# shyam196/egc

Measured on AMD Instinct MI355X. Metric: EGC-M layer fwd edges/sec on ogbn-arxiv; achieved HBM GB/s vs roofline, higher is better.
Workload: dtype f32; 1 GPU; ogbn-arxiv-shaped full graph: N=169343, heavy-tailed symmetrised E_in=2329056 (+N self loops => E_eff=2498399), EGC-M d=128 H=8 B=4 aggrs=sum+mean+max+symnorm, CSR cached; n_nodes=169343, e_in=2329056, e_eff=2498399, layer=EGConv, parallelism=single GPU

## Files before the change

egc_amd/_C.py:

```python
from __future__ import annotations

import ctypes as C
import os

_LIB_PATH = os.environ.get("EGC_HIP_LIB") or os.path.join(os.path.dirname(os.path.abspath(__file__)), "lib",
                                                         "libegc_hip.so")
_lib = None

EGC_MAX_AGGRS = 8
LONG_ROW_THRESHOLD = 64
LONG_ROW_CHUNK = 256

AGGR_SUM, AGGR_MEAN, AGGR_MAX, AGGR_MIN, AGGR_VAR, AGGR_STD, AGGR_SYMNORM = range(7)
SET_RAW, SET_LOOPED = 0, 1
LAYOUT_HBA, LAYOUT_HAB = 0, 1
ACT_NONE, ACT_SOFTMAX, ACT_SIGMOID, ACT_HARDTANH = range(4)
READOUT_SUM, READOUT_MEAN, READOUT_MAX = range(3)
SOFTMAX_MAX_CLASSES = 1024
TYPED_MAX_RELATIONS = 8
TOKEN_HEAD_MAX_SEQ = 8
TOKEN_HEAD_SLAB = 64
TOKEN_HEAD_MAX_IN = 384
MPNN_ADD, MPNN_MEAN, MPNN_MAX = range(3)
PNA_SUM, PNA_MEAN, PNA_MIN, PNA_MAX, PNA_VAR, PNA_STD = range(6)
PNA_IDENTITY, PNA_AMPLIFICATION, PNA_ATTENUATION, PNA_LINEAR, PNA_INVERSE_LINEAR = range(5)
NBR_SUM, NBR_MEAN, NBR_MEAN_T, NBR_SYM = range(4)

_STATUS = {1: "EGC_ERR_INVALID", 2: "EGC_ERR_WORKSPACE", 3: "EGC_ERR_HIP", 4: "EGC_ERR_UNSUPPORTED"}


class EgcGraph(C.Structure):
    _fields_ = [
        ("n_nodes", C.c_int64), ("n_edges", C.c_int64),
        ("rowptr", C.c_void_p), ("col", C.c_void_p), ("edge_id", C.c_void_p),
        ("dis_raw", C.c_void_p), ("dis_looped", C.c_void_p),
        ("max_index", C.c_void_p), ("plan", C.c_void_p), ("n_chunks", C.c_int64),
        ("n_src_rows", C.c_int64), ("edge_dis_raw", C.c_void_p), ("edge_dis_looped", C.c_void_p),
    ]


class EgcLayer(C.Structure):
    _fields_ = [
        ("in_channels", C.c_int32), ("out_channels", C.c_int32), ("num_heads", C.c_int32),
        ("num_bases", C.c_int32), ("num_aggrs", C.c_int32), ("aggrs", C.c_int32 * EGC_MAX_AGGRS),
        ("agg_set", C.c_int32), ("sym_set", C.c_int32), ("loops_all_nodes", C.c_int32),
        ("weight_layout", C.c_int32), ("weight_act", C.c_int32), ("basis_stride", C.c_int32),
    ]


_ENV_DATA = getattr(os.environ, "_data", None)


def env_flag(name: str) -> bool:
    if _ENV_DATA is not None:
        v = _ENV_DATA.get(name.encode())
        return v is not None and v not in (b"", b"0")
    return os.environ.get(name, "0") not in ("", "0")


class EgcPost(C.Structure):
    _fields_ = [("scale", C.c_void_p), ("shift", C.c_void_p), ("residual", C.c_void_p), ("relu", C.c_int32)]


class EgcTypedRel(C.Structure):
    _fields_ = [("rowptr", C.c_void_p), ("col", C.c_void_p), ("pre_rowptr", C.c_void_p), ("in_", C.c_void_p),
                ("n_edges", C.c_int64), ("n_in_rows", C.c_int64), ("ld_in", C.c_int32), ("out_col", C.c_int32),
                ("post_mean", C.c_int32), ("reserved", C.c_int32)]


SYMBOLS = {
    "egc_plan_ints": (C.c_int64, [C.c_int64, C.c_int64]),
    "egc_coo_to_csr_workspace_bytes": (C.c_size_t, [C.c_int64, C.c_int64]),
    "egc_coo_to_csr": (C.c_int, [C.c_void_p, C.c_void_p, C.c_int64, C.c_int64, C.c_void_p, C.c_void_p,
                                 C.c_void_p, C.c_void_p, C.c_void_p, C.c_size_t, C.c_void_p]),
    "egc_coo_to_csr_checked": (C.c_int, [C.c_void_p, C.c_void_p, C.c_int64, C.c_int64, C.c_int64, C.c_void_p, C.c_void_p,
                                         C.c_void_p, C.c_void_p, C.c_void_p, C.c_void_p, C.c_void_p, C.c_size_t, C.c_void_p]),
    "egc_graph_build_workspace_bytes": (C.c_size_t, [C.c_int64, C.c_int64]),
    "egc_graph_build_scratch_bytes": (C.c_size_t, [C.c_int64]),
    "egc_graph_build": (C.c_int, [C.c_void_p, C.c_void_p, C.c_int64, C.c_int64, C.c_int64, C.c_void_p, C.c_void_p, C.c_void_p,
                                  C.c_void_p, C.c_void_p, C.c_void_p, C.c_void_p, C.c_void_p, C.c_void_p, C.c_void_p,
                                  C.c_void_p, C.c_void_p, C.c_size_t, C.c_void_p, C.c_size_t, C.c_void_p]),
    "egc_csr_edge_dis": (C.c_int, [C.c_int64, C.c_void_p, C.c_void_p, C.c_void_p, C.c_void_p, C.c_void_p, C.c_void_p]),
    "egc_csr_prepare": (C.c_int, [C.c_int64, C.c_int64, C.c_void_p, C.c_void_p, C.c_void_p, C.c_void_p,
                                  C.c_void_p, C.c_void_p]),
    "egc_bases_ld": (C.c_int32, [C.POINTER(EgcLayer)]),
    "egc_basis_transform_f32": (C.c_int, [C.c_void_p, C.c_void_p, C.c_void_p, C.c_int64, C.c_int32, C.c_int32,
                                          C.c_int32, C.c_void_p, C.c_int32, C.c_void_p, C.c_void_p]),
    "egc_basis_pack_bytes": (C.c_size_t, [C.c_int32, C.c_int32, C.c_int32]),
    "egc_basis_pack": (C.c_int, [C.c_void_p, C.c_int32, C.c_int32, C.c_int32, C.c_void_p, C.c_size_t, C.c_void_p]),
    "egc_layer_gemm_flags": (C.c_int32, [C.POINTER(EgcLayer)]),
    "egc_basis_pack_ex": (C.c_int, [C.c_void_p, C.c_int32, C.c_int32, C.c_int32, C.c_int32, C.c_void_p, C.c_size_t, C.c_void_p]),
    "egc_basis_transform_packed_ex": (C.c_int, [C.c_void_p, C.c_void_p, C.c_void_p, C.c_int64, C.c_int32, C.c_int32,
                                                C.c_int32, C.c_int32, C.c_void_p, C.c_int32, C.c_void_p, C.c_void_p]),
    "egc_basis_transform_packed_add": (C.c_int, [C.c_void_p, C.c_void_p, C.c_void_p, C.c_int64, C.c_int32, C.c_int32,
                                                 C.c_int32, C.c_int32, C.c_void_p, C.c_void_p, C.c_int32, C.c_void_p, C.c_void_p]),
    "egc_basis_pack_transposed": (C.c_int, [C.c_void_p, C.c_int64, C.c_int32, C.c_int32, C.c_int32, C.c_void_p, C.c_size_t,
                                            C.c_void_p]),
    "egc_basis_transform_packed": (C.c_int, [C.c_void_p, C.c_void_p, C.c_void_p, C.c_int64, C.c_int32, C.c_int32,
                                             C.c_int32, C.c_void_p, C.c_int32, C.c_void_p, C.c_void_p]),
    "egc_layer_forward_packed": (C.c_int, [C.POINTER(EgcGraph), C.POINTER(EgcLayer), C.c_void_p, C.c_void_p,
                                           C.c_void_p, C.c_void_p, C.c_void_p, C.c_int32, C.c_void_p, C.c_void_p,
                                           C.c_void_p, C.c_size_t, C.c_void_p]),
    "egc_aggregate_workspace_bytes": (C.c_size_t, [C.POINTER(EgcLayer), C.c_int64, C.c_int64]),
    "egc_aggregate_workspace_zero_bytes": (C.c_size_t, [C.POINTER(EgcLayer), C.c_int64, C.c_int64]),
    "egc_aggregate_workspace_bytes_for": (C.c_size_t, [C.POINTER(EgcLayer), C.POINTER(EgcGraph)]),
    "egc_aggregate_combine_f32": (C.c_int, [C.POINTER(EgcGraph), C.POINTER(EgcLayer), C.c_void_p, C.c_int32,
                                            C.c_void_p, C.c_void_p, C.c_void_p, C.c_void_p, C.c_void_p,
                                            C.c_void_p, C.c_size_t, C.c_void_p]),
    "egc_layer_forward_f32": (C.c_int, [C.POINTER(EgcGraph), C.POINTER(EgcLayer), C.c_void_p, C.c_void_p,
                                        C.c_void_p, C.c_void_p, C.c_void_p, C.c_int32, C.c_void_p, C.c_void_p,
                                        C.c_void_p, C.c_size_t, C.c_void_p]),
    "egc_backward_workspace_bytes": (C.c_size_t, [C.POINTER(EgcLayer), C.c_int64]),
    "egc_backward_workspace_bytes_for": (C.c_size_t, [C.POINTER(EgcLayer), C.POINTER(EgcGraph)]),
    "egc_aggregate_combine_rows_f32": (C.c_int, [C.POINTER(EgcGraph), C.POINTER(EgcLayer), C.c_void_p, C.c_int32,
                                                 C.c_void_p, C.c_void_p, C.c_void_p, C.c_int64, C.c_int64,
                                                 C.c_void_p, C.c_size_t, C.c_void_p]),
    "egc_aggregate_combine_post_f32": (C.c_int, [C.POINTER(EgcGraph), C.POINTER(EgcLayer), C.c_void_p, C.c_int32,
                                                 C.c_void_p, C.c_void_p, C.POINTER(EgcPost), C.c_void_p,
                                                 C.c_void_p, C.c_size_t, C.c_void_p]),
    "egc_aggregate_combine_strided_f32": (C.c_int, [C.POINTER(EgcGraph), C.POINTER(EgcLayer), C.c_void_p, C.c_int32,
                                                    C.c_void_p, C.c_int32, C.c_void_p, C.POINTER(EgcPost), C.c_void_p,
                                                    C.c_void_p, C.c_size_t, C.c_void_p]),
    "egc_weight_grad_workspace_bytes": (C.c_int64, [C.c_int64, C.c_int32, C.c_int32]),
    "egc_weight_grad_plan": (C.c_int, [C.c_int64, C.c_int32, C.c_int32, C.c_void_p]),
    "egc_weight_grad_ex_workspace_bytes": (C.c_int64, [C.c_int64, C.c_int32, C.c_int32, C.c_int32]),
    "egc_weight_grad_ex_f32": (C.c_int, [C.c_void_p, C.c_int64, C.c_void_p, C.c_int64, C.c_int64, C.c_int32, C.c_int32,
                                         C.c_void_p, C.c_void_p, C.c_void_p, C.c_int64, C.c_int32, C.c_void_p, C.c_void_p,
                                         C.c_int64, C.c_void_p]),
    "egc_weight_grad_params_f32": (C.c_int, [C.c_void_p, C.c_int64, C.c_void_p, C.c_int64, C.c_int64, C.c_int32, C.c_int32, C.c_int32,
                                             C.c_int32, C.c_int32, C.c_int32, C.c_int32, C.c_void_p, C.c_int32, C.c_void_p,
                                             C.c_void_p, C.c_void_p, C.c_void_p, C.c_int64, C.c_int32, C.c_void_p, C.c_void_p,
                                             C.c_int64, C.c_void_p]),
    "egc_weight_grad_f32": (C.c_int, [C.c_void_p, C.c_int64, C.c_void_p, C.c_int64, C.c_int64, C.c_int32, C.c_int32,
                                      C.c_void_p, C.c_void_p, C.c_void_p, C.c_int64, C.c_void_p]),
    "egc_csr_transposed_coo": (C.c_int, [C.c_int64, C.c_int64, C.c_void_p, C.c_void_p, C.c_void_p, C.c_void_p, C.c_void_p]),
    "egc_column_moments_f64": (C.c_int, [C.c_void_p, C.c_void_p, C.c_void_p, C.c_void_p, C.c_int32, C.c_void_p, C.c_float,
                                         C.c_int64, C.c_int32, C.c_void_p, C.c_int32, C.c_void_p, C.c_void_p, C.c_void_p]),
    "egc_bn_forward_stats_f32": (C.c_int, [C.c_void_p, C.c_int64, C.c_int32, C.c_void_p, C.c_int32, C.c_void_p, C.c_void_p, C.c_void_p,
                                           C.c_void_p, C.c_double, C.c_void_p, C.c_void_p, C.c_void_p, C.c_void_p, C.c_double,
                                           C.c_void_p, C.c_void_p, C.c_void_p]),
    "egc_bn_backward_stats_f32": (C.c_int, [C.c_void_p, C.c_void_p, C.c_void_p, C.c_void_p, C.c_int32, C.c_void_p, C.c_float, C.c_int64,
                                            C.c_int32, C.c_void_p, C.c_int32, C.c_void_p, C.c_void_p, C.c_void_p, C.c_void_p,
                                            C.c_void_p, C.c_void_p]),
    "egc_bn_backward_stats_sums_f32": (C.c_int, [C.c_void_p, C.c_void_p, C.c_void_p, C.c_void_p, C.c_int32, C.c_void_p, C.c_float, C.c_int64,
                                                 C.c_int32, C.c_void_p, C.c_int32, C.c_void_p, C.c_void_p, C.c_void_p, C.c_void_p,
                                                 C.c_void_p, C.c_void_p, C.c_void_p]),
    "egc_bn_forward_finalize": (C.c_int, [C.c_void_p, C.c_int32, C.c_int32, C.c_int64, C.c_void_p, C.c_void_p, C.c_double,
                                          C.c_void_p, C.c_void_p, C.c_void_p, C.c_void_p, C.c_double, C.c_void_p, C.c_void_p,
                                          C.c_void_p]),
    "egc_bn_backward_finalize": (C.c_int, [C.c_void_p, C.c_int32, C.c_int32, C.c_int64, C.c_void_p, C.c_void_p, C.c_void_p,
                                           C.c_void_p, C.c_void_p]),
    "egc_affine_act_residual_f32": (C.c_int, [C.c_void_p, C.c_void_p, C.c_void_p, C.c_void_p, C.c_int32, C.c_void_p, C.c_float,
                                              C.c_int64, C.c_int32, C.c_void_p, C.c_void_p, C.c_void_p]),
    "egc_affine_act_backward_f32": (C.c_int, [C.c_void_p, C.c_void_p, C.c_void_p, C.c_void_p, C.c_int32, C.c_void_p, C.c_float,
                                              C.c_void_p, C.c_void_p, C.c_void_p, C.c_int64, C.c_int32, C.c_void_p,
                                              C.c_void_p, C.c_void_p]),
    "egc_weights_pack_f32": (C.c_int, [C.c_void_p, C.c_int32, C.c_void_p, C.c_void_p, C.c_int32, C.c_int32, C.c_int32,
                                       C.c_int32, C.c_int32, C.c_int32, C.c_int32, C.c_void_p, C.c_void_p, C.c_int32,
                                       C.c_void_p]),
    "egc_sum_partials_f32": (C.c_int, [C.c_void_p, C.c_int32, C.c_int32, C.c_void_p, C.c_void_p]),
    "egc_column_sums_f32": (C.c_int, [C.c_void_p, C.c_int64, C.c_int32, C.c_int32, C.c_void_p, C.c_int32, C.c_void_p]),
    "egc_segment_mean_f32": (C.c_int, [C.c_void_p, C.c_void_p, C.c_int64, C.c_int32, C.c_void_p, C.c_void_p]),
    "egc_segment_reduce_f32": (C.c_int, [C.c_void_p, C.c_void_p, C.c_int64, C.c_int64, C.c_int32, C.c_int32, C.c_void_p,
                                         C.c_void_p, C.c_void_p]),
    "egc_segment_reduce_backward_f32": (C.c_int, [C.c_void_p, C.c_void_p, C.c_void_p, C.c_int64, C.c_int64, C.c_int32,
# ... 169 lines not shown
```

egc_amd/csrc/egc_aggregate.hip:

```cpp
#include <stdlib.h>

#include <algorithm>

#include "egc_aggregate_host.h"
#include "egc_fused_tile_host.h"
#include "egc_gemm_split.h"
#include "egc_pack_map.h"

namespace egc {

bool stdvar_reference(const egc_layer* layer) {
  const char* e = getenv("EGC_STDVAR_REFERENCE");
  if (layer == nullptr || e == nullptr || e[0] == '\0' || (e[0] == '0' && e[1] == '\0')) return false;
  for (int t = 0; t < layer->num_aggrs && t < EGC_MAX_AGGRS; ++t)
    if (layer->aggrs[t] == EGC_AGGR_VAR || layer->aggrs[t] == EGC_AGGR_STD) return true;
  return false;
}

template <int CHUNKS>
__device__ inline void set_shift(const AggArgs& a, __amdgpu_buffer_rsrc_t rsrc, int row, int lane, Acc<CHUNKS>& acc) {
  bool need = false;
  for (int t = 0; t < a.A; ++t) need = need || a.aggr[t] == EGC_AGGR_VAR || a.aggr[t] == EGC_AGGR_STD;
  if (!need && a.stats == nullptr) return;
  if (a.var_ref) return;
// ... 502 lines not shown

int egc_aggregate_combine_rows_f32(const egc_graph* graph, const egc_layer* layer, const float* bases, int32_t ldb,
                                   const float* weightings, const float* bias, float* out, int64_t row_begin,
                                   int64_t row_end, void* workspace, size_t workspace_bytes, egc_stream_t stream) {
  if (row_end < 0) return EGC_ERR_INVALID;
  return aggregate_combine_impl(graph, layer, bases, ldb, weightings, bias, nullptr, out, nullptr, nullptr, row_begin,
                                row_end, workspace, workspace_bytes, stream);
}

int egc_aggregate_combine_post_f32(const egc_graph* graph, const egc_layer* layer, const float* bases, int32_t ldb,
                                   const float* weightings, const float* bias, const egc_post* post, float* out,
                                   void* workspace, size_t workspace_bytes, egc_stream_t stream) {
  if (post != nullptr && ((post->scale == nullptr) != (post->shift == nullptr))) return EGC_ERR_INVALID;
  return aggregate_combine_impl(graph, layer, bases, ldb, weightings, bias, post, out, nullptr, nullptr, 0, -1, workspace,
                                workspace_bytes, stream);
}

int egc_aggregate_combine_strided_f32(const egc_graph* graph, const egc_layer* layer, const float* bases, int32_t ldb,
                                      const float* weightings, int32_t ldw, const float* bias, const egc_post* post,
                                      float* out, void* workspace, size_t workspace_bytes, egc_stream_t stream) {
  if (post != nullptr && ((post->scale == nullptr) != (post->shift == nullptr))) return EGC_ERR_INVALID;
  return aggregate_combine_impl(graph, layer, bases, ldb, weightings, bias, post, out, nullptr, nullptr, 0, -1, workspace,
                                workspace_bytes, stream, nullptr, nullptr, nullptr, ldw);
}

int egc_aggregate_combine_train_f32(const egc_graph* graph, const egc_layer* layer, const float* bases, int32_t ldb,
                                    const float* weightings, const float* bias, float* out, float* stats,
                                    int32_t* cnt, int32_t* arg_max, int32_t* arg_min, void* workspace,
                                    size_t workspace_bytes, egc_stream_t stream) {
  if (graph == nullptr || layer == nullptr || stats == nullptr || cnt == nullptr) return EGC_ERR_INVALID;
  bool arg_done = false;
  int st = aggregate_combine_impl(graph, layer, bases, ldb, weightings, bias, nullptr, out, stats, cnt, 0, -1, workspace,
                                  workspace_bytes, stream, arg_max, arg_min, &arg_done);
  if (st != EGC_OK || arg_done) return st;
  unsigned *a8max, *a8min;
  arg8_tables(layer, graph->n_nodes, stats, arg_max != nullptr, arg_min != nullptr, &a8max, &a8min);
  return egc::arg_extrema(graph, layer, bases, ldb, stats, cnt, arg_max, arg_min, a8max, a8min, (hipStream_t)stream);
}

int egc_aggregate_combine_train_rows_f32(const egc_graph* graph, const egc_layer* layer, const float* bases, int32_t ldb,
                                         const float* weightings, const float* bias, float* out, float* stats,
                                         int32_t* cnt, int32_t* arg_max, int32_t* arg_min, int64_t row_begin,
                                         int64_t row_end, void* workspace, size_t workspace_bytes, egc_stream_t stream) {
  if (graph == nullptr || layer == nullptr || stats == nullptr || cnt == nullptr || row_end < 0) return EGC_ERR_INVALID;
  bool arg_done = false;
  int st = aggregate_combine_impl(graph, layer, bases, ldb, weightings, bias, nullptr, out, stats, cnt, row_begin, row_end,
                                  workspace, workspace_bytes, stream, arg_max, arg_min, &arg_done);
  if (st != EGC_OK || arg_done || row_end < graph->n_nodes) return st;
  unsigned *a8max, *a8min;
  arg8_tables(layer, graph->n_nodes, stats, arg_max != nullptr, arg_min != nullptr, &a8max, &a8min);
  return egc::arg_extrema(graph, layer, bases, ldb, stats, cnt, arg_max, arg_min, a8max, a8min, (hipStream_t)stream);
}

static int aggregate_combine_impl(const egc_graph* graph, const egc_layer* layer, const float* bases, int32_t ldb,
                                  const float* weightings, const float* bias, const egc_post* post, float* out,
                                  float* stats, int32_t* cnt_out, int64_t row_begin, int64_t row_end, void* workspace,
                                  size_t workspace_bytes, egc_stream_t stream_, int32_t* arg_max, int32_t* arg_min,
                                  bool* arg_done, int32_t ldw) {
  hipStream_t stream = (hipStream_t)stream_;
  if (graph == nullptr) return EGC_ERR_INVALID;
  int st = validate_layer(layer);
  if (st != EGC_OK) return st;
  const int64_t n = graph->n_nodes, e = graph->n_edges;
  if (n < 0 || e < 0 || n >= ((int64_t)1 << 31) - 1 || e >= ((int64_t)1 << 31) - 1) return EGC_ERR_INVALID;
  if (n == 0) return EGC_OK;
  if (graph->rowptr == nullptr || graph->plan == nullptr || (e > 0 && graph->col == nullptr)) return EGC_ERR_INVALID;
  if (bases == nullptr || weightings == nullptr || out == nullptr) return EGC_ERR_INVALID;
  if (ldb != egc_bases_ld(layer)) return EGC_ERR_INVALID;
  if ((reinterpret_cast<uintptr_t>(bases) & 15) != 0) return EGC_ERR_INVALID;
  const int64_t n_src = graph->n_src_rows > 0 ? graph->n_src_rows : n;
  if (n_src < n && (layer->agg_set == EGC_SET_LOOPED || layer_uses_symnorm(layer))) return EGC_ERR_INVALID;
  if ((uint64_t)n_src * (uint64_t)ldb * 4ull > (uint64_t)OOB) return EGC_ERR_UNSUPPORTED;

  AggArgs a;
  a.rowptr = graph->rowptr;
  a.col = graph->col;
  a.dis = nullptr;
  a.edis = nullptr;
  if (layer_uses_symnorm(layer)) {
    a.dis = layer->sym_set == EGC_SET_LOOPED ? graph->dis_looped : graph->dis_raw;
    a.edis = layer->sym_set == EGC_SET_LOOPED ? graph->edge_dis_looped : graph->edge_dis_raw;
    if (a.dis == nullptr) return EGC_ERR_INVALID;
  }
  a.max_index = graph->max_index;
  if (layer->loops_all_nodes == 0 && graph->max_index == nullptr) return EGC_ERR_INVALID;
  a.plan = graph->plan;
  a.bases = bases;
  a.weightings = weightings;
  a.bias = bias;
  a.out = out;
  a.n_nodes = (int)n;
  a.l4_off = 0;
  a.wide_p0 = a.wide_p1 = 0;
  a.row_begin = (int)row_begin;
  a.row_end = row_end < 0 ? (int)n : (int)row_end;
  if (a.row_begin < 0 || a.row_end > (int)n) return EGC_ERR_INVALID;
  if (a.row_begin >= a.row_end) return EGC_OK;
  agg_layer_fields(layer, a);
  if (ldw > 0) a.ldw = ldw;
  if (a.ldw != a.W && (a.ldw < a.W || (a.ldw & 3) != 0 || (reinterpret_cast<uintptr_t>(weightings) & 15) != 0))
    return EGC_ERR_INVALID;
  a.magic_L = a.L > 1 ? agg_magic(a.L) : 0u;
  a.bases_bytes = (unsigned)((uint64_t)n_src * ldb * 4ull);
  agg_set_post(a, post);
  a.stats = stats;
  a.cnt_out = cnt_out;
  a.stat_k = stat_layout(a.aggr, a.A, a.stat_slot);
  a.arg_max = a.stat_slot[STAT_MX] >= 0 ? arg_max : nullptr;
  a.arg_min = a.stat_slot[STAT_MN] >= 0 ? arg_min : nullptr;
  a.arg8_max = a.arg8_min = nullptr;
  if (stats != nullptr) arg8_tables(layer, n, stats, a.arg_max != nullptr, a.arg_min != nullptr, &a.arg8_max, &a.arg8_min);
  a.self_pos = (int)e;

  a.var_ref = stdvar_reference(layer) ? 1 : 0;
  int chunks = 1;
  if (a.slots <= 64) {
    int lg = 0;
    while ((1 << lg) < a.slots) ++lg;
    a.lpr_log2 = a.var_ref ? 6 : lg;
  } else {
    a.lpr_log2 = 6;
    chunks = (a.slots + 63) / 64;
  }
  a.lds_floats_per_wave = a.A * ldb + ((a.W + 3) & ~3);
  int wpb = 4;
  if ((size_t)wpb * a.lds_floats_per_wave * sizeof(float) > 40 * 1024) wpb = 1;
  const size_t lds_bytes = (size_t)wpb * a.lds_floats_per_wave * sizeof(float);
  if (lds_bytes > 64 * 1024) return EGC_ERR_UNSUPPORTED;

  WsLayout w = ws_layout(layer, n, e, graph->n_chunks);
  if (workspace == nullptr || workspace_bytes < w.total) return EGC_ERR_WORKSPACE;
  a.counters = (int*)workspace;
  a.queue = (int*)((char*)workspace + w.counter_bytes);
  a.partial = (float*)((char*)workspace + w.counter_bytes + w.queue_bytes);
  a.partial_nself = (int*)((char*)workspace + w.counter_bytes + w.queue_bytes + w.partial_bytes);
  a.x = nullptr;
  a.F_in = layer->in_channels;
  a.M = 0;
  a.wfrag = nullptr;
  a.wbias4 = nullptr;
  PlanCaps caps = plan_caps(n, e);
  a.rows_per_wave = 0;
  a.n_chunks_hint = (graph->n_chunks >= 0 && graph->n_chunks <= caps.cap_chunks) ? (int)graph->n_chunks : -1;
  const bool force_generic = getenv("EGC_FORCE_GENERIC") != nullptr || a.var_ref != 0;
  if (!force_generic && fast_path_supported(a, layer->weight_layout, chunks)) {
    if (arg_done != nullptr) *arg_done = true;
    return launch_fast(a, n, caps, stream);
  }

  switch (chunks) {
    case 1: return launch_all<1>(a, n, caps, wpb, lds_bytes, stream);
    case 2: return launch_all<2>(a, n, caps, wpb, lds_bytes, stream,
                                 !force_generic && getenv("EGC_NO_WIDE") == nullptr && wide_path_supported(a, layer->weight_layout));
    case 3: return launch_all<3>(a, n, caps, wpb, lds_bytes, stream);
    case 4: return launch_all<4>(a, n, caps, wpb, lds_bytes, stream);
    default: return EGC_ERR_UNSUPPORTED;
  }
}

int egc_layer_forward_f32(const egc_graph* graph, const egc_layer* layer, const float* x, const float* wcat,
                          const float* bcat, const float* bias, float* bases, int32_t ldb, float* weightings,
                          float* out, void* workspace, size_t workspace_bytes, egc_stream_t stream) {
  if (graph == nullptr) return EGC_ERR_INVALID;
  int st = validate_layer(layer);
  if (st != EGC_OK) return st;
  const int fg = layer->num_bases * layer_basis_stride(layer);
// ... 302 lines not shown
```

egc_amd/csrc/egc_aggregate_dev.h:

```cpp
#pragma once
#include <math.h>

#include "egc_common.h"

#pragma clang fp contract(off)

namespace egc {

template <class I>
__device__ inline I half_wave_lower_bound(const int64_t* __restrict__ arr, I n, int64_t key, int lane) {
  const int l32 = lane & 31, sh = lane & 32;
  I lo = 0, hi = n;
  while (__ballot(hi - lo > 32) != 0) {
    const bool live = hi - lo > 32;
    const I step = live ? (hi - lo + 31) / 32 : 1;
    const I i = lo + (I)l32 * step;
    const bool ge = (live && i < hi) ? arr[i] >= key : true;
    const unsigned m = (unsigned)(__ballot(ge) >> sh);
    if (!live) continue;
    const int f = __ffs((int)m) - 1;
    if (f < 0) { lo = lo + 31 * step + 1; if (lo > hi) lo = hi; continue; }
    const I nhi = lo + (I)f * step;
    lo = f > 0 ? lo + (I)(f - 1) * step + 1 : lo;
    hi = nhi < hi ? nhi : hi;
  }
  const I i = lo + l32;
  const bool ge = i < hi ? arr[i] >= key : true;
  const unsigned m = (unsigned)(__ballot(ge) >> sh);
  const int f = __ffs((int)m) - 1;
  return f < 0 ? hi : (lo + f < hi ? lo + f : hi);
}

constexpr unsigned ARG8_NONE = 254u, ARG8_FAR = 255u;
__device__ inline unsigned arg8_pack(int4 a, int start, int n_edges) {
  auto enc = [&](int p) -> unsigned {
    if (p < 0 || p >= n_edges) return ARG8_NONE;
    const unsigned rel = (unsigned)(p - start);
    return rel < ARG8_NONE ? rel : ARG8_FAR;
  };
  return enc(a.x) | (enc(a.y) << 8) | (enc(a.z) << 16) | (enc(a.w) << 24);
}

struct AggArgs {
  const int* rowptr;
  const int* col;
  const float* dis;
  const float* edis;
  const int* max_index;
  const int* plan;
  const float* bases;
  const float* weightings;
  const float* bias;
  float* out;
  float* partial;
  int* partial_nself;
  int* counters;
  int n_nodes;
  int row_begin, row_end;
  int ldb, slots;
  int F_out, W, H, B, A, L;
  int ldw;
  int Ls;
  int aggr[EGC_MAX_AGGRS];
  int x_looped, y_looped, loops_all;
  int sa, sb;
  int act;
  int lpr_log2;
  unsigned magic_L;
  unsigned bases_bytes;
  int lds_floats_per_wave;
  int lpb_log2;
  int lanes_pb;
  unsigned magic_P;
  unsigned magic_P1;
  int hpg;
  int rows_per_wave;
  int chunk_blocks;
  int need_mean, need_var;
  int var_ref;
  int n_chunks_hint;
  int l4_off;
  int wide_p0, wide_p1;
  int w_lds_stride;
  int bias_lds_floats;
  const float* post_scale;
  const float* post_shift;
  const float* residual;
  int post_relu;
  float* stats;
  int* cnt_out;
  int stat_slot[5];
  int stat_k;
  int* arg_max;
  int* arg_min;
  unsigned* arg8_max;
  unsigned* arg8_min;
  int self_pos;
  int w_aw;
  const float* x;
  const float* wfrag;
  const float* wbias4;
  int F_in, M;
  int* queue;
};


template <int CHUNKS>
struct Acc {
  f4 sum[CHUNKS], sq[CHUNKS], mx[CHUNKS], mn[CHUNKS], ws[CHUNKS];
  f4 sh[CHUNKS];
  __device__ inline void init() {
#pragma unroll
    for (int k = 0; k < CHUNKS; ++k) {
      sum[k] = 0.f; sq[k] = 0.f; ws[k] = 0.f; sh[k] = 0.f;
      mx[k] = -INFINITY; mn[k] = INFINITY;
    }
  }
};

__device__ inline f4 f4_max(f4 a, f4 b) {
  return f4{fmaxf(a.x, b.x), fmaxf(a.y, b.y), fmaxf(a.z, b.z), fmaxf(a.w, b.w)};
}
__device__ inline f4 f4_min(f4 a, f4 b) {
  return f4{fminf(a.x, b.x), fminf(a.y, b.y), fminf(a.z, b.z), fminf(a.w, b.w)};
}
__device__ inline f4 f4_fma(f4 a, f4 b, f4 c) {
  return f4{fmaf(a.x, b.x, c.x), fmaf(a.y, b.y, c.y), fmaf(a.z, b.z, c.z), fmaf(a.w, b.w, c.w)};
}
__device__ inline f4 f4_shfl_xor(f4 v, int off) {
  return f4{__shfl_xor(v.x, off), __shfl_xor(v.y, off), __shfl_xor(v.z, off), __shfl_xor(v.w, off)};
}

__device__ inline f4 load_slot(__amdgpu_buffer_rsrc_t rsrc, unsigned byte_off) {
  return __builtin_bit_cast(f4, __builtin_amdgcn_raw_buffer_load_b128(rsrc, byte_off, 0, 0));
}

__device__ inline void fold(f4& sum, f4& sq, f4& mx, f4& mn, f4& ws, f4 v, bool in_x, bool in_y, float w, f4 sh) {
  const f4 vx = in_x ? v : f4{0.f, 0.f, 0.f, 0.f};
  sum += vx;
  const f4 d = in_x ? v - sh : f4{0.f, 0.f, 0.f, 0.f};
  sq += f4{__fmul_rn(d.x, d.x), __fmul_rn(d.y, d.y), __fmul_rn(d.z, d.z), __fmul_rn(d.w, d.w)};
  mx = f4_max(mx, in_x ? v : f4{-INFINITY, -INFINITY, -INFINITY, -INFINITY});
  mn = f4_min(mn, in_x ? v : f4{INFINITY, INFINITY, INFINITY, INFINITY});
  const float wy = in_y ? w : 0.f;
  ws = f4_fma(f4{wy, wy, wy, wy}, v, ws);
}


__device__ inline f4 f4_div(f4 a, float d) { return f4{a.x / d, a.y / d, a.z / d, a.w / d}; }

__device__ inline f4 f4_var(f4 mean_sq, f4 mean) {
  return f4{__fsub_rn(mean_sq.x, __fmul_rn(mean.x, mean.x)), __fsub_rn(mean_sq.y, __fmul_rn(mean.y, mean.y)),
            __fsub_rn(mean_sq.z, __fmul_rn(mean.z, mean.z)), __fsub_rn(mean_sq.w, __fmul_rn(mean.w, mean.w))};
}
__device__ inline f4 f4_std(f4 var) {
  return f4{sqrtf(fmaxf(var.x, 0.f) + 1e-5f), sqrtf(fmaxf(var.y, 0.f) + 1e-5f), sqrtf(fmaxf(var.z, 0.f) + 1e-5f),
            sqrtf(fmaxf(var.w, 0.f) + 1e-5f)};
}

__device__ inline __amdgpu_buffer_rsrc_t bases_rsrc(const AggArgs& a) {
  return __builtin_amdgcn_make_buffer_rsrc((void*)a.bases, 0, a.bases_bytes, 0x00020000);
}

bool fast_path_supported(const AggArgs& a, int layout, int chunks);
int launch_fast(AggArgs a, int64_t n_nodes, const PlanCaps& caps, hipStream_t stream);
bool wide_path_supported(const AggArgs& a, int layout);
int launch_wide_rows(AggArgs a, const PlanCaps& caps, hipStream_t stream);

constexpr int FUSEDW_QUEUE_INTS = 16;

int tile_capacity(AggArgs a, int tmax, int emax, bool with_post);
int launch_tile_plan(const int64_t* ptr, int64_t n_graphs, const int64_t* dst, int64_t n_edges, int64_t n_nodes, int slot,
                     int n_slots, int4* tiles, int* count, const int64_t* edge_ptr, hipStream_t stream);
int launch_tile_simple(AggArgs a, const int4* tiles, const int* n_tiles_dev, int n_tiles_bound, int tlds, int tmax, int emax,
                       const int64_t* src, const int64_t* dst, const int* max_index, int32_t* status, int32_t* host_flag,
                       hipStream_t stream);

struct FtPlan;
FtPlan fused_tile_plan(const AggArgs& a, int f_in, bool with_post, bool bwd);
int fused_tile_pack(const FtPlan& p, const AggArgs& a, const float* wcat, const float* bcat, int f_in, void* packed, hipStream_t stream);
int launch_fused_tile(AggArgs a, const int64_t* ptr, const int64_t* edge_ptr, int64_t n_graphs, const int64_t* src,
                      const int64_t* dst, int64_t n_edges, const int* max_index, const float* x, int f_in, const void* packed,
                      int tcap, int emax, int32_t* status, int32_t* host_flag, hipStream_t stream);

int fused_tile_bwd_pack(const FtPlan& pb, const AggArgs& a, const float* wcat, int f_in, void* packed_t, hipStream_t stream);
struct PackPtrs;
struct PackDims;
int fused_tile_train_pack_params(const FtPlan& pb, const AggArgs& a, const PackPtrs& bases, const float* comb_w, const float* comb_b,
                                 const float* bcat, const PackDims& d, void* packed, void* packed_t, hipStream_t stream);
int fused_tile_train_pack(const FtPlan& pb, const AggArgs& a, const float* wcat, const float* bcat, int f_in, void* packed, void* packed_t,
                          hipStream_t stream);
int launch_fused_tile_bwd(AggArgs a, const int64_t* ptr, const int64_t* edge_ptr, int64_t n_graphs, const int64_t* src,
                          const int64_t* dst, int64_t n_edges, const int* max_index, const float* x, int f_in, const void* packed,
                          const void* packed_t, const float* grad_out, float* d_x, const float* d_x_add, float* d_cat, int ld_dcat, int tcap, int emax,
                          int32_t* status, int32_t* host_flag, hipStream_t stream);

}
```

egc_amd/csrc/egc_aggregate_fast.hip:

```cpp
#include <stdlib.h>

#include "egc_aggregate_host.h"

namespace egc {

template <int LPR_LOG2, int HPB, int NEED, class C>
#ifndef EGC_AGG_WAVES_SQ
#define EGC_AGG_WAVES_SQ 5
#endif
__global__ void __launch_bounds__(256) __attribute__((amdgpu_waves_per_eu(NEED == 0 ? EGC_AGG_WAVES : ((NEED & NEED_ARG) && (NEED & NEED_SQ)) ? 2 : (NEED == NEED_SQ || NEED == NEED_MN) ? EGC_AGG_WAVES_SQ : 4)))
agg_fast_kernel(AggArgs a) {
  constexpr int LPR = 1 << LPR_LOG2, G = 64 / LPR;
  extern __shared__ float smem[];
  if ((int)blockIdx.x < a.chunk_blocks && (int)blockIdx.x * 4 >= a.plan[1]) return;
  const int wave = __builtin_amdgcn_readfirstlane(threadIdx.x >> 6);
  const int lane = threadIdx.x & 63;
  const int g = lane >> LPR_LOG2;
  const int q = lane & (LPR - 1);
  const unsigned slot_off = (unsigned)q * 16u;
  const unsigned row_bytes = (unsigned)a.ldb * 4u;
  const bool lane_live = q < C::slots(a);
  const int F_out = C::F_out(a);
  float* lds_bias = smem + wave * a.lds_floats_per_wave;
  const bool post = a.post_scale != nullptr;
  float* lds_scale = lds_bias + a.bias_lds_floats;
  float* lds_w = lds_bias + (post ? 2 : 1) * a.bias_lds_floats;
  for (int o = lane; o < C::H(a) * C::Ls(a); o += 64) {
    const int h = o / C::Ls(a), l = o - h * C::Ls(a);
    const int c = h * C::L(a) + l;
    const bool real = l < C::L(a);
    float bv = (a.bias != nullptr && real) ? a.bias[c] : 0.f;
    if (post) {
      const float sc = real ? a.post_scale[c] : 0.f;
      bv = fmaf(bv, sc, real ? a.post_shift[c] : 0.f);
      lds_scale[o] = sc;
    }
    lds_bias[o] = bv;
  }
  asm volatile("s_waitcnt lgkmcnt(0)" ::: "memory");
  FastRsrc R;
  R.bases = bases_rsrc(a);
  R.out = __builtin_amdgcn_make_buffer_rsrc((void*)a.out, 0, (unsigned)a.n_nodes * (unsigned)F_out * 4u, 0x00020000);
  R.res = __builtin_amdgcn_make_buffer_rsrc((void*)(a.residual != nullptr ? a.residual : a.out), 0,
                                            (unsigned)a.n_nodes * (unsigned)F_out * 4u, 0x00020000);
  const bool looped_any = C::xl(a) || C::yl(a);

  if ((int)blockIdx.x < a.chunk_blocks) {
    const int c = __builtin_amdgcn_readfirstlane(blockIdx.x * 4 + wave);
    long_row_chunk<LPR_LOG2, HPB, NEED, C>(a, R, c, lane, lds_w, lds_bias, lds_scale);
    return;
  }

  const int Q = a.rows_per_wave;
  const int gw = ((int)blockIdx.x - a.chunk_blocks) * 4 + wave;
  const int r0 = __builtin_amdgcn_readfirstlane(a.row_begin + gw * Q * G);
  const int n_end = a.row_end;
  if (r0 >= n_end) return;
  const int rp = a.rowptr[min(r0 + lane, a.n_nodes)];
  const int grp_addr = (g << LPR_LOG2) << 2;
  int start_n = bperm(g << 2, rp);
  int nd_n;
  {
    const int deg = bperm((g + 1) << 2, rp) - start_n;
    nd_n = (r0 + g < n_end && deg <= EGC_LONG_ROW_THRESHOLD) ? deg : 0;
  }
  int jj_n = q < nd_n ? a.col[start_n + q] : 0;
  for (int k = 0; k < Q; ++k) {
    const int rbase = r0 + k * G;
    if (rbase >= n_end) break;
    const int row = rbase + g;
    const bool row_ok = row < n_end;
    const int start = start_n, nd = nd_n;
    int jj = jj_n;
    if (k + 1 < Q) {
      start_n = bperm(((k + 1) * G + g) << 2, rp);
      const int deg = bperm(((k + 1) * G + g + 1) << 2, rp) - start_n;
      nd_n = (rbase + G + g < n_end && deg <= EGC_LONG_ROW_THRESHOLD) ? deg : 0;
      jj_n = q < nd_n ? a.col[start_n + q] : 0;
    }
    int maxd = nd;
#pragma unroll
    for (int off = LPR; off < 64; off <<= 1) maxd = max(maxd, bperm((lane ^ off) << 2, maxd));
    maxd = __builtin_amdgcn_readfirstlane(maxd);
    f4 wpre[2], vself;
    bool has_self;
    const float dis_i = (a.dis != nullptr && row_ok) ? a.dis[row] : 0.f;
    load_row_operands<LPR_LOG2, C>(a, R, lane, row, row_ok, wpre, vself, has_self);

    FAcc<NEED> acc;
    acc.init();
    if constexpr (NEED & NEED_SQ) {
      const int first = bperm(grp_addr, jj);
      acc.sh = load_slot(R.bases, (lane_live && nd > 0) ? (unsigned)first * row_bytes + slot_off : OOB);
    }
    int nself = 0;
    for (int ts = 0; ts < maxd; ts += LPR) {
      if (ts > 0) jj = (ts + q < nd) ? a.col[start + ts + q] : 0;
      const bool pv = ts + q < nd;
      const float dd = !pv ? 0.f : a.edis != nullptr ? a.edis[start + ts + q] : a.dis != nullptr ? a.dis[jj] : 0.f;
      if (looped_any) {
        const unsigned long long sb = __ballot(pv && jj == row);
        nself += __popcll((sb >> (g << LPR_LOG2)) & ((LPR == 64) ? ~0ull : ((1ull << LPR) - 1ull)));
      }
      const int cnt = min(LPR, maxd - ts);
      for (int t0 = 0; t0 < cnt; t0 += FU)
        gather_batch<NEED, C>(a, R, acc, grp_addr + (t0 << 2), 4, row, jj, dd, dis_i, lane_live ? nd : 0, ts + t0, 1, row_bytes,
                              slot_off, start);
    }
    int ln = lane;
    asm volatile("" : "+v"(ln));
    const int deg_all = bperm((k * G + g + 1) << 2, rp) - start;
    const bool is_short = deg_all <= EGC_LONG_ROW_THRESHOLD;
    finish_group<LPR_LOG2, HPB, NEED, C>(a, R, ln, row, row_ok, acc, nd, nself, dis_i, vself, has_self, wpre, is_short,
                                         lds_w, lds_bias, lds_scale);
  }
}

constexpr int WFU = 2;

template <class Base, int SET, int PS = 0, int OFF = 0>
struct WideSet : Base {
  static constexpr bool stat = PS > 0;
  static __device__ inline int lanes_pb(const AggArgs& a) { return stat ? PS : (SET == 0 ? a.wide_p0 : a.wide_p1); }
  static __device__ inline int slots(const AggArgs& a) { return Base::B(a) * lanes_pb(a); }
  static __device__ inline bool pow2(const AggArgs& a) { return stat ? ((PS & (PS - 1)) == 0 && (Base::B(a) & (Base::B(a) - 1)) == 0) : false; }
  static __device__ inline int lpb_log2(const AggArgs&) { return stat ? ilog2(PS > 0 ? PS : 1) : -1; }
  static __device__ inline int basis_of(const AggArgs& a, int q) {
    return stat ? q / (PS > 0 ? PS : 1) : (int)__umulhi((unsigned)q, SET == 0 ? a.magic_P : a.magic_P1);
  }
  static __device__ inline int l4_off(const AggArgs& a) { return stat ? OFF : (SET == 0 ? 0 : a.wide_p0); }
};

struct WideLane {
  bool live0, live1;
  unsigned so0, so1;
};

template <class C0, class C1>
__device__ inline WideLane wide_lane(const AggArgs& a, int lane) {
  WideLane w;
  const int P = a.Ls >> 2, B = C0::B(a);
  const int b0 = min(C0::basis_of(a, lane), B - 1), b1 = min(C1::basis_of(a, lane), B - 1);
  w.live0 = lane < C0::slots(a);
  w.live1 = lane < C1::slots(a);
  w.so0 = (unsigned)(b0 * P + (lane - b0 * C0::lanes_pb(a))) * 16u;
  w.so1 = (unsigned)(b1 * P + C1::l4_off(a) + (lane - b1 * C1::lanes_pb(a))) * 16u;
  return w;
}

template <int NEED, class C0>
__device__ inline void wide_gather(const AggArgs& a, const FastRsrc& R, const WideLane& wl_, FAcc<NEED>& acc0, FAcc<NEED>& acc1,
                                   int row, int jj, float dd, float dis_i, int cnt, unsigned row_bytes, int pos_base) {
  for (int t0 = 0; t0 < cnt; t0 += WFU) {
    f4 v0[WFU], v1[WFU];
    float w[WFU];
    bool in_x[WFU];
#pragma unroll
    for (int u = 0; u < WFU; ++u) {
      const int addr = (t0 + u) << 2;
      const int j = bperm(addr, jj);
      const bool is_self = j == row;
      in_x[u] = (t0 + u < cnt) && !(C0::xl(a) && is_self);
      const unsigned base = (unsigned)j * row_bytes;
      v0[u] = load_slot(R.bases, (in_x[u] && wl_.live0) ? base + wl_.so0 : OOB);
      v1[u] = load_slot(R.bases, (in_x[u] && wl_.live1) ? base + wl_.so1 : OOB);
      w[u] = bperm(addr, dd) * dis_i;
      if (C0::yl(a) && !C0::xl(a)) w[u] = is_self ? 0.f : w[u];
    }
#pragma unroll
    for (int u = 0; u < WFU; ++u) {
      fold<NEED>(acc0, v0[u], w[u], in_x[u] && wl_.live0, pos_base + t0 + u);
      fold<NEED>(acc1, v1[u], w[u], in_x[u] && wl_.live1, pos_base + t0 + u);
    }
  }
}

template <int HPB, int NEED, class C0, class C1>
__device__ inline void wide_finish(const AggArgs& a, const FastRsrc& R, const WideLane& wl_, int lane, int row, FAcc<NEED>& acc0,
                                   FAcc<NEED>& acc1, int deg, int nself, float dis_i, unsigned row_bytes, float* lds_w,
                                   const float* lds_bias, const float* lds_scale) {
  const bool looped_any = C0::xl(a) || C0::yl(a);
  const bool has_self = C0::loops_all(a) || row <= *a.max_index;
// ... 172 lines not shown
      const int first = __builtin_amdgcn_readfirstlane(jj);
      acc0.sh = load_slot(R.bases, (wl_.live0 && deg > 0) ? (unsigned)first * row_bytes + wl_.so0 : OOB);
      acc1.sh = load_slot(R.bases, (wl_.live1 && deg > 0) ? (unsigned)first * row_bytes + wl_.so1 : OOB);
    }
    wide_gather<NEED, C0>(a, R, wl_, acc0, acc1, row, jj, dd, dis_i, deg, row_bytes, start);
    wide_finish<HPB, NEED, C0, C1>(a, R, wl_, lane, row, acc0, acc1, deg, nself, dis_i, row_bytes, lds_w, lds_bias, lds_scale);
  }
}

bool wide_path_supported(const AggArgs& a, int layout) {
  if (layout != EGC_LAYOUT_HBA || a.act == EGC_ACT_SOFTMAX) return false;
  if (a.x_looped && !a.y_looped) return false;
  if (a.slots <= 64 || a.slots > 128) return false;
  if ((a.Ls & 3) != 0 || a.ldb != a.B * a.Ls) return false;
  if ((a.B & (a.B - 1)) != 0) return false;
  if (a.A < 1 || a.A > AMAX) return false;
  if (agg_hpb(a) > HPB_MAX) return false;
  if (a.W > 512) return false;
  const int P = a.Ls / 4, P0 = (P + 1) / 2;
  if (a.B * P0 > 64) return false;
  if (a.stats != nullptr || a.arg_max != nullptr || a.arg_min != nullptr) return false;
  if ((uint64_t)a.n_nodes * (uint64_t)a.F_out * 4ull > (uint64_t)OOB) return false;
  if ((size_t)4 * agg_strip_floats(a, 1, a.post_scale != nullptr) * sizeof(float) > 64 * 1024) return false;
  return true;
}

template <int HPB, int NEED, class C0, class C1>
static int launch_wide_one(const AggArgs& a, unsigned grid, size_t lds, hipStream_t stream) {
  agg_wide_kernel<HPB, NEED, C0, C1><<<grid, 256, lds, stream>>>(a);
  EGC_LAUNCH_CHECK("agg_wide_kernel");
  return EGC_OK;
}

template <class St, int HPB, int NEED, int P0, int P1>
static bool try_wide_static(const AggArgs& a, unsigned grid, size_t lds, hipStream_t stream, int* status) {
  if (!cfg_matches<St>(a)) return false;
  *status = launch_wide_one<HPB, NEED, WideSet<St, 0, P0, 0>, WideSet<St, 1, P1, P0>>(a, grid, lds, stream);
  return true;
}

int launch_wide_rows(AggArgs a, const PlanCaps& caps, hipStream_t stream) {
  const int P = a.Ls / 4;
  a.wide_p0 = (P + 1) / 2;
  a.wide_p1 = P - a.wide_p0;
  agg_lane_geometry(a, a.wide_p0);
  a.lpb_log2 = -1;
  a.magic_P1 = agg_magic(a.wide_p1);
  a.l4_off = 0;
  a.rows_per_wave = 8;
  a.chunk_blocks = (int)ceil_div(a.n_chunks_hint >= 0 ? a.n_chunks_hint : caps.cap_chunks, 4);
  const int need = agg_need(a);
  agg_lds_strips(a, 1, a.post_scale != nullptr);
  const size_t lds = (size_t)4 * a.lds_floats_per_wave * sizeof(float);
  if (lds > 64 * 1024) return EGC_ERR_UNSUPPORTED;
  const unsigned grid = (unsigned)(a.chunk_blocks + ceil_div((int64_t)a.row_end - a.row_begin, (int64_t)4 * a.rows_per_wave));
  if (getenv("EGC_NO_STATIC_CFG") == nullptr) {
    int status = EGC_OK;
    constexpr int X = EGC_AGGR_MAX, N = EGC_AGGR_MIN, Y = EGC_AGGR_SYMNORM;
    if (try_wide_static<StCfg<4, 4, 75, 3, agg_pack(Y, N, X), EGC_ACT_NONE, false, true, true, 76>, 1, NEED_MN, 10, 9>(
            a, grid, lds, stream, &status)) return status;
    if (try_wide_static<StCfg<8, 8, 38, 1, agg_pack(Y), EGC_ACT_NONE, false, true, true, 40>, 1, 0, 5, 5>(
            a, grid, lds, stream, &status)) return status;
  }
  using R0 = WideSet<RtCfg, 0>;
  using R1 = WideSet<RtCfg, 1>;
  return agg_dispatch_rows<NeedCoarse>(a, need, [&](auto hpb, auto nd) {
    return launch_wide_one<decltype(hpb)::value, decltype(nd)::value, R0, R1>(a, grid, lds, stream);
  });
}

bool fast_path_supported(const AggArgs& a, int layout, int chunks) {
  if (chunks != 1 || layout != EGC_LAYOUT_HBA || a.act == EGC_ACT_SOFTMAX) return false;
  if (a.x_looped && !a.y_looped) return false;
  if (a.slots < 1 || a.slots > 64) return false;
  if ((a.Ls & 3) != 0 || a.ldb != a.B * a.Ls) return false;
  if ((a.B & (a.B - 1)) != 0) return false;
  if (a.A < 1 || a.A > AMAX) return false;
  if (agg_hpb(a) > HPB_MAX) return false;
  if (a.W > 8 * agg_lpr(a.slots)) return false;
  if ((uint64_t)a.n_nodes * (uint64_t)a.F_out * 4ull > (uint64_t)OOB) return false;
  return true;
}

template <int LPR_LOG2, int HPB, int NEED, class C>
static int launch_one(const AggArgs& a, unsigned grid, size_t lds, hipStream_t stream) {
  agg_fast_kernel<LPR_LOG2, HPB, NEED, C><<<grid, 256, lds, stream>>>(a);
  EGC_LAUNCH_CHECK("agg_fast_kernel");
  return EGC_OK;
}

template <class C, int NEED>
static bool try_static(const AggArgs& a, unsigned grid, size_t lds, hipStream_t stream, int* status) {
  constexpr int LPR_LOG2 = agg_lpr_log2(C::kB * C::P_), HPB = (C::kH + C::kB - 1) / C::kB;
  if (!cfg_matches<C>(a) || a.slots > (1 << LPR_LOG2) || 2 * a.slots <= (1 << LPR_LOG2)) return false;
  if constexpr (C::has(EGC_AGGR_MAX)) {
    if (a.arg_max != nullptr) {
      *status = launch_one<LPR_LOG2, HPB, NEED | NEED_ARG, C>(a, grid, lds, stream);
      return true;
    }
  }
  *status = launch_one<LPR_LOG2, HPB, NEED, C>(a, grid, lds, stream);
  return true;
}

#define EGC_STATIC_CFG(H, B, L, A, AGG, ACT, XL, YL, LA, NEED)                                                      \
  if (try_static<StCfg<H, B, L, A, AGG, ACT, XL, YL, LA, ((L) + 3) / 4 * 4>, NEED>(a, grid, lds, stream, &status)) \
    return status;

int launch_fast(AggArgs a, int64_t n_nodes, const PlanCaps& caps, hipStream_t stream) {
  const int G = 64 / agg_lpr(a.slots);
  agg_lane_geometry(a);
  if (a.rows_per_wave <= 0) a.rows_per_wave = (G == 1 && (int64_t)a.row_end - a.row_begin >= 32768) ? 4 : 1;
  if (a.rows_per_wave * G > 60) a.rows_per_wave = 60 / G;
  a.chunk_blocks = (int)ceil_div(a.n_chunks_hint >= 0 ? a.n_chunks_hint : caps.cap_chunks, 4);
  const int need = agg_need(a);
  agg_lds_strips(a, G, a.post_scale != nullptr);
  size_t lds = (size_t)4 * a.lds_floats_per_wave * sizeof(float);
  if (lds > 64 * 1024) return EGC_ERR_UNSUPPORTED;
  const int64_t row_blocks = ceil_div((int64_t)a.row_end - a.row_begin, (int64_t)4 * a.rows_per_wave * G);
  const unsigned grid = (unsigned)(a.chunk_blocks + row_blocks);

  if (getenv("EGC_NO_STATIC_CFG") == nullptr) {
    int status = EGC_OK;
    constexpr int S = EGC_AGGR_SUM, M = EGC_AGGR_MEAN, X = EGC_AGGR_MAX, Y = EGC_AGGR_SYMNORM;
    EGC_STATIC_CFG(8, 4, 16, 4, agg_pack(S, M, X, Y), EGC_ACT_NONE, true, true, true, 0)
    EGC_STATIC_CFG(8, 4, 16, 3, agg_pack(S, X, Y), EGC_ACT_NONE, true, true, true, 0)
    EGC_STATIC_CFG(8, 4, 16, 4, agg_pack(S, EGC_AGGR_STD, X, Y), EGC_ACT_NONE, true, true, true, NEED_SQ)
    EGC_STATIC_CFG(8, 4, 16, 1, agg_pack(Y), EGC_ACT_NONE, true, true, true, 0)
    EGC_STATIC_CFG(8, 4, 16, 3, agg_pack(Y, X, M), EGC_ACT_NONE, false, true, true, 0)
    EGC_STATIC_CFG(8, 4, 16, 1, agg_pack(Y), EGC_ACT_NONE, false, true, true, 0)
    EGC_STATIC_CFG(8, 4, 23, 1, agg_pack(Y), EGC_ACT_NONE, false, true, true, 0)
    EGC_STATIC_CFG(4, 4, 34, 3, agg_pack(Y, X, M), EGC_ACT_NONE, false, true, true, 0)
    EGC_STATIC_CFG(8, 4, 21, 1, agg_pack(Y), EGC_ACT_NONE, false, true, true, 0)
    EGC_STATIC_CFG(4, 4, 31, 3, agg_pack(S, EGC_AGGR_STD, X), EGC_ACT_NONE, false, true, true, NEED_SQ)
    EGC_STATIC_CFG(4, 4, 32, 3, agg_pack(Y, EGC_AGGR_STD, X), EGC_ACT_NONE, false, true, true, NEED_SQ)
    EGC_STATIC_CFG(8, 4, 37, 1, agg_pack(Y), EGC_ACT_NONE, false, true, true, 0)
    EGC_STATIC_CFG(4, 4, 56, 3, agg_pack(S, M, X), EGC_ACT_NONE, false, true, true, 0)
    EGC_STATIC_CFG(8, 4, 44, 1, agg_pack(Y), EGC_ACT_NONE, true, true, true, 0)
    EGC_STATIC_CFG(8, 4, 44, 1, agg_pack(M), EGC_ACT_NONE, true, true, true, 0)
    EGC_STATIC_CFG(8, 4, 16, 2, agg_pack(M, X), EGC_ACT_NONE, false, false, true, 0)
    EGC_STATIC_CFG(8, 4, 16, 1, agg_pack(S), EGC_ACT_NONE, false, false, true, 0)
    EGC_STATIC_CFG(4, 4, 16, 2, agg_pack(M, X), EGC_ACT_NONE, false, false, true, 0)
    EGC_STATIC_CFG(4, 4, 16, 1, agg_pack(S), EGC_ACT_NONE, false, false, true, 0)
  }
  return agg_dispatch<NeedFine>(a, need, [&](auto lpr, auto hpb, auto nd) {
    return launch_one<decltype(lpr)::value, decltype(hpb)::value, decltype(nd)::value, RtCfg>(a, grid, lds, stream);
  });
}

}
```

egc_amd/csrc/egc_aggregate_fast_dev.h:

```cpp
#pragma once
#include <stdlib.h>

#include "egc_aggregate_dev.h"

namespace egc {

constexpr int OUT_NT = 2;
#ifndef EGC_AGG_FU
#define EGC_AGG_FU 4
#endif
constexpr int FU = EGC_AGG_FU;
constexpr int HPB_MAX = 4;
#ifndef EGC_AGG_WAVES
#define EGC_AGG_WAVES 6
#endif

constexpr int NEED_SQ = 1;
constexpr int NEED_MN = 2;
constexpr int NEED_ARG = 4;
constexpr int ARG_NONE = 0x7fffffff;

struct RtCfg {
  static constexpr int kH = 0;
  static __device__ inline int H(const AggArgs& a) { return a.H; }
// ... 177 lines not shown
        "v"(p3.w));
  return p0;
}

template <int NEED>
struct FAcc {
  f4 sum, mx, ws;
  f4 sq, mn;
  f4 sh;
  i4 ax, an;
  __device__ inline void init() {
    sum = 0.f; ws = 0.f; mx = -INFINITY;
    if constexpr (NEED & NEED_SQ) { sq = 0.f; sh = 0.f; }
    if constexpr (NEED & NEED_MN) mn = INFINITY;
    if constexpr (NEED & NEED_ARG) ax = an = ARG_NONE;
  }
};

__device__ inline void take_gt4(f4& m, i4& ar, f4 v, int pos) {
  const bool cx = v.x > m.x, cy = v.y > m.y, cz = v.z > m.z, cw = v.w > m.w;
  m = f4{cx ? v.x : m.x, cy ? v.y : m.y, cz ? v.z : m.z, cw ? v.w : m.w};
  ar = i4{cx ? pos : ar.x, cy ? pos : ar.y, cz ? pos : ar.z, cw ? pos : ar.w};
}
__device__ inline void take_lt4(f4& m, i4& ar, f4 v, int pos) {
  const bool cx = v.x < m.x, cy = v.y < m.y, cz = v.z < m.z, cw = v.w < m.w;
  m = f4{cx ? v.x : m.x, cy ? v.y : m.y, cz ? v.z : m.z, cw ? v.w : m.w};
  ar = i4{cx ? pos : ar.x, cy ? pos : ar.y, cz ? pos : ar.z, cw ? pos : ar.w};
}
__device__ inline void merge_gt4(f4& m, i4& ar, f4 om, i4 oa) {
  const bool cx = om.x > m.x || (om.x == m.x && oa.x < ar.x), cy = om.y > m.y || (om.y == m.y && oa.y < ar.y);
  const bool cz = om.z > m.z || (om.z == m.z && oa.z < ar.z), cw = om.w > m.w || (om.w == m.w && oa.w < ar.w);
  m = f4{cx ? om.x : m.x, cy ? om.y : m.y, cz ? om.z : m.z, cw ? om.w : m.w};
  ar = i4{cx ? oa.x : ar.x, cy ? oa.y : ar.y, cz ? oa.z : ar.z, cw ? oa.w : ar.w};
}
__device__ inline void merge_lt4(f4& m, i4& ar, f4 om, i4 oa) {
  const bool cx = om.x < m.x || (om.x == m.x && oa.x < ar.x), cy = om.y < m.y || (om.y == m.y && oa.y < ar.y);
  const bool cz = om.z < m.z || (om.z == m.z && oa.z < ar.z), cw = om.w < m.w || (om.w == m.w && oa.w < ar.w);
  m = f4{cx ? om.x : m.x, cy ? om.y : m.y, cz ? om.z : m.z, cw ? om.w : m.w};
  ar = i4{cx ? oa.x : ar.x, cy ? oa.y : ar.y, cz ? oa.z : ar.z, cw ? oa.w : ar.w};
}

template <int NEED>
__device__ inline void fold(FAcc<NEED>& acc, f4 v, float w, bool in_x, int pos) {
  acc.sum += v;
  acc.ws = f4_fma(splat(w), v, acc.ws);
  if (in_x) {
    if constexpr (NEED & NEED_SQ) acc.sq += f4_sqr_rn(v - acc.sh);
    if constexpr (NEED & NEED_ARG) {
      take_gt4(acc.mx, acc.ax, v, pos);
      if constexpr (NEED & NEED_MN) take_lt4(acc.mn, acc.an, v, pos);
    } else {
      acc.mx = f4_vmax(acc.mx, v);
      if constexpr (NEED & NEED_MN) acc.mn = f4_vmin(acc.mn, v);
    }
  }
}

template <int LPR_LOG2, int NEED>
__device__ inline void all_reduce_groups(FAcc<NEED>& acc, int lane) {
#pragma unroll
  for (int off = 1 << LPR_LOG2; off < 64; off <<= 1) {
    const int addr = (lane ^ off) << 2;
    acc.sum += bperm(addr, acc.sum);
    acc.ws += bperm(addr, acc.ws);
    if constexpr (NEED & NEED_SQ) acc.sq += bperm(addr, acc.sq);
    if constexpr (NEED & NEED_ARG) {
      merge_gt4(acc.mx, acc.ax, bperm(addr, acc.mx), bperm(addr, acc.ax));
      if constexpr (NEED & NEED_MN) merge_lt4(acc.mn, acc.an, bperm(addr, acc.mn), bperm(addr, acc.an));
    } else {
      acc.mx = f4_vmax(acc.mx, bperm(addr, acc.mx));
      if constexpr (NEED & NEED_MN) acc.mn = f4_vmin(acc.mn, bperm(addr, acc.mn));
    }
  }
}

__device__ inline f4 load_slot_wt(__amdgpu_buffer_rsrc_t rsrc, unsigned byte_off) {
  return __builtin_bit_cast(f4, __builtin_amdgcn_raw_buffer_load_b128(rsrc, byte_off, 0, 0x11));
}

struct FastRsrc {
  __amdgpu_buffer_rsrc_t bases, out, res;
};

template <int NEED, class C>
__device__ inline void gather_batch(const AggArgs& a, const FastRsrc& R, FAcc<NEED>& acc, int addr0, int step, int row,
                                    int jj, float dd, float dis_i, int n_valid, int first, int vstep,
                                    unsigned row_bytes, unsigned slot_off, int pos_base) {
  f4 v[FU];
  float w[FU];
  bool in_x[FU];
#pragma unroll
  for (int u = 0; u < FU; ++u) {
    const int addr = addr0 + u * step;
    const int j = bperm(addr, jj);
    const bool is_self = j == row;
    in_x[u] = (first + u * vstep < n_valid) && !(C::xl(a) && is_self);
    v[u] = load_slot(R.bases, in_x[u] ? (unsigned)j * row_bytes + slot_off : OOB);
    w[u] = bperm(addr, dd) * dis_i;
    if (C::yl(a) && !C::xl(a)) w[u] = is_self ? 0.f : w[u];
  }
#pragma unroll
  for (int u = 0; u < FU; ++u) fold<NEED>(acc, v[u], w[u], in_x[u], pos_base + first + u * vstep);
}

template <int LPR_LOG2, int HPB, int NEED, class C, bool W_READY = false, int W_AW = 4>
__device__ inline void finish_group(const AggArgs& a, const FastRsrc& R, int lane, int row, bool row_ok, FAcc<NEED>& acc,
                                    int deg, int nself, float dis_i, f4 vself, bool has_self, const f4 (&wpre)[2],
                                    bool store, float* lds_w, const float* lds_bias, const float* lds_scale) {
  constexpr int LPR = 1 << LPR_LOG2;
  const int g = lane >> LPR_LOG2;
  const int q = lane & (LPR - 1);
  const int A = C::A(a), B = C::B(a), H = C::H(a), W = C::W(a);
  int b, l4;
  const bool live = q < C::slots(a);
  if (C::pow2(a)) {
    b = min(q >> C::lpb_log2(a), B - 1);
    l4 = q & ((1 << C::lpb_log2(a)) - 1);
  } else {
    b = min(C::basis_of(a, q), B - 1);
    l4 = q - b * C::lanes_pb(a);
  }

  float* wl = lds_w + g * a.w_lds_stride;
  const int AW = W_READY ? (W_AW > 0 ? W_AW : a.w_aw) : A;
#pragma unroll
  for (int k = 0; k < 2; ++k) {
    const int c0 = (q + k * LPR) * 4;
    if (!W_READY && c0 < W) {
      f4 t = wpre[k];
      if (C::act(a) == EGC_ACT_SIGMOID) {
        t = f4{1.0f / (1.0f + expf(-t.x)), 1.0f / (1.0f + expf(-t.y)), 1.0f / (1.0f + expf(-t.z)),
               1.0f / (1.0f + expf(-t.w))};
      } else if (C::act(a) == EGC_ACT_HARDTANH) {
        t = f4{fminf(fmaxf(t.x, -1.f), 1.f), fminf(fmaxf(t.y, -1.f), 1.f), fminf(fmaxf(t.z, -1.f), 1.f),
               fminf(fmaxf(t.w, -1.f), 1.f)};
      }
      *reinterpret_cast<f4*>(wl + c0) = t;
    }
  }

  int cnt = deg;
  if (C::xl(a)) cnt = deg - nself + (has_self ? 1 : 0);
  if (C::xl(a)) {
    fold<NEED>(acc, vself, dis_i * dis_i, has_self, a.self_pos);
  } else if (C::yl(a)) {
    acc.ws = f4_fma(splat(dis_i * dis_i), vself, acc.ws);
  }
  if (a.stats != nullptr && store && row_ok && live) {
    float* st = a.stats + ((int64_t)row * a.stat_k) * a.ldb + 4 * q;
    if (a.stat_slot[STAT_SUM] >= 0) __builtin_nontemporal_store(acc.sum, reinterpret_cast<f4*>(st + a.stat_slot[STAT_SUM] * a.ldb));
    if (a.stat_slot[STAT_MX] >= 0) __builtin_nontemporal_store(acc.mx, reinterpret_cast<f4*>(st + a.stat_slot[STAT_MX] * a.ldb));
    if (a.stat_slot[STAT_WS] >= 0) __builtin_nontemporal_store(acc.ws, reinterpret_cast<f4*>(st + a.stat_slot[STAT_WS] * a.ldb));
    if constexpr (NEED & NEED_SQ)
      if (a.stat_slot[STAT_SQ] >= 0) {
        const float cf = (float)max(cnt, 1);
        const f4 ds = f4_fma(splat(-(float)cnt), acc.sh, acc.sum);
        __builtin_nontemporal_store(f4_var(f4_div(acc.sq, cf), f4_div(ds, cf)), reinterpret_cast<f4*>(st + a.stat_slot[STAT_SQ] * a.ldb));
      }
    if constexpr (NEED & NEED_MN)
      if (a.stat_slot[STAT_MN] >= 0) __builtin_nontemporal_store(acc.mn, reinterpret_cast<f4*>(st + a.stat_slot[STAT_MN] * a.ldb));
    if (q == 0) a.cnt_out[row] = cnt;
    if constexpr (NEED & NEED_ARG) {
      const int none = cnt > 0 ? a.self_pos : -1;
      const int64_t ao = (int64_t)row * a.ldb + 4 * q;
      if (a.arg_max != nullptr) {
        const i4 r = i4{acc.ax.x == ARG_NONE ? none : acc.ax.x, acc.ax.y == ARG_NONE ? none : acc.ax.y,
                        acc.ax.z == ARG_NONE ? none : acc.ax.z, acc.ax.w == ARG_NONE ? none : acc.ax.w};
        __builtin_nontemporal_store(r, reinterpret_cast<i4*>(a.arg_max + ao));
        if (a.arg8_max != nullptr)
          __builtin_nontemporal_store(arg8_pack(int4{r.x, r.y, r.z, r.w}, a.rowptr[row], a.self_pos), a.arg8_max + (ao >> 2));
      }
      if constexpr (NEED & NEED_MN)
        if (a.arg_min != nullptr) {
          const i4 r = i4{acc.an.x == ARG_NONE ? none : acc.an.x, acc.an.y == ARG_NONE ? none : acc.an.y,
                          acc.an.z == ARG_NONE ? none : acc.an.z, acc.an.w == ARG_NONE ? none : acc.an.w};
          __builtin_nontemporal_store(r, reinterpret_cast<i4*>(a.arg_min + ao));
          if (a.arg8_min != nullptr)
            __builtin_nontemporal_store(arg8_pack(int4{r.x, r.y, r.z, r.w}, a.rowptr[row], a.self_pos), a.arg8_min + (ao >> 2));
        }
    }
// ... 99 lines not shown
          part += bperm(((g << LPR_LOG2) + (live ? src : q)) << 2, part);
        }
      } else if (LPR == 16 && C::lpb_log2(a) == 2 && C::slots(a) == 16) {
        dpp_sum_over_4_bases(part);
      } else {
        for (int off = 1 << C::lpb_log2(a); off < C::slots(a); off <<= 1) part += bperm((lane ^ off) << 2, part);
      }
      if (b == bb) o[hb] = part;
    }
  }
  l4 += C::l4_off(a);
  const unsigned orow = (unsigned)row * (unsigned)C::F_out(a) * 4u;
#pragma unroll
  for (int hb = 0; hb < HPB; ++hb) {
    const int h = hb * B + b;
    const bool mine = store && row_ok && live && h < H;
    const int oc = h * C::L(a) + 4 * l4;
    if (!C::padded(a)) {
      f4 r = o[hb];
      if (a.post_scale != nullptr) r = r * *reinterpret_cast<const f4*>(lds_scale + (mine ? oc : 0));
      r = r + *reinterpret_cast<const f4*>(lds_bias + (mine ? oc : 0));
      if (a.post_relu) r = f4{fmaxf(r.x, 0.f), fmaxf(r.y, 0.f), fmaxf(r.z, 0.f), fmaxf(r.w, 0.f)};
      if (a.residual != nullptr) r = r + load_slot(R.res, mine ? orow + (unsigned)oc * 4u : OOB);
      __builtin_amdgcn_raw_buffer_store_b128(__builtin_bit_cast(u32x4, r), R.out, mine ? orow + (unsigned)oc * 4u : OOB, 0, OUT_NT);
    } else {
      f4 r = o[hb];
      if (a.post_scale != nullptr) r = r * *reinterpret_cast<const f4*>(lds_scale + (mine ? h * C::Ls(a) + 4 * l4 : 0));
      r = r + *reinterpret_cast<const f4*>(lds_bias + (mine ? h * C::Ls(a) + 4 * l4 : 0));
      if (a.post_relu) r = f4{fmaxf(r.x, 0.f), fmaxf(r.y, 0.f), fmaxf(r.z, 0.f), fmaxf(r.w, 0.f)};
      const int left = mine ? C::L(a) - 4 * l4 : 0;
      const unsigned base = orow + (unsigned)oc * 4u;
      float rx = r.x, ry = r.y, rz = r.z, rw = r.w;
      if (a.residual != nullptr) {
        const float* rr = a.residual + (int64_t)(mine ? row : 0) * C::F_out(a) + (mine ? oc : 0);
        rx += left > 0 ? rr[0] : 0.f; ry += left > 1 ? rr[1] : 0.f; rz += left > 2 ? rr[2] : 0.f; rw += left > 3 ? rr[3] : 0.f;
      }
      __builtin_amdgcn_raw_buffer_store_b32(__float_as_uint(rx), R.out, left > 0 ? base : OOB, 0, OUT_NT);
      __builtin_amdgcn_raw_buffer_store_b32(__float_as_uint(ry), R.out, left > 1 ? base + 4u : OOB, 0, OUT_NT);
      __builtin_amdgcn_raw_buffer_store_b32(__float_as_uint(rz), R.out, left > 2 ? base + 8u : OOB, 0, OUT_NT);
      __builtin_amdgcn_raw_buffer_store_b32(__float_as_uint(rw), R.out, left > 3 ? base + 12u : OOB, 0, OUT_NT);
    }
  }
  asm volatile("s_waitcnt lgkmcnt(0)" ::: "memory");
}

template <int LPR_LOG2, class C, bool NO_W = false>
__device__ inline void load_row_operands(const AggArgs& a, const FastRsrc& R, int lane, int row, bool row_ok,
                                         f4 (&wpre)[2], f4& vself, bool& has_self) {
  constexpr int LPR = 1 << LPR_LOG2;
  const int q = lane & (LPR - 1);
  const int W = C::W(a);
  has_self = row_ok && (C::loops_all(a) || row <= *a.max_index);
  const bool want_self = (C::xl(a) || C::yl(a)) && has_self;
  vself = load_slot(R.bases, (want_self && q < C::slots(a)) ? (unsigned)row * (unsigned)a.ldb * 4u + (unsigned)q * 16u : OOB);
  if (NO_W) {
    wpre[0] = wpre[1] = f4{0.f, 0.f, 0.f, 0.f};
    return;
  }
  const float* wrow = a.weightings + (int64_t)(row_ok ? row : a.row_begin) * a.ldw;
#pragma unroll
  for (int k = 0; k < 2; ++k) {
    const int c0 = (q + k * LPR) * 4;
    wpre[k] = f4{0.f, 0.f, 0.f, 0.f};
    if (c0 + 3 < W) wpre[k] = __builtin_nontemporal_load(reinterpret_cast<const f4*>(wrow + c0));
    else if (c0 < W) {
      wpre[k].x = wrow[c0];
      if (c0 + 1 < W) wpre[k].y = wrow[c0 + 1];
      if (c0 + 2 < W) wpre[k].z = wrow[c0 + 2];
    }
  }
}



template <class C>
__device__ inline f4 w_act(const AggArgs& a, f4 t) {
  if (C::act(a) == EGC_ACT_SIGMOID)
    return f4{1.0f / (1.0f + expf(-t.x)), 1.0f / (1.0f + expf(-t.y)), 1.0f / (1.0f + expf(-t.z)), 1.0f / (1.0f + expf(-t.w))};
  if (C::act(a) == EGC_ACT_HARDTANH)
    return f4{fminf(fmaxf(t.x, -1.f), 1.f), fminf(fmaxf(t.y, -1.f), 1.f), fminf(fmaxf(t.z, -1.f), 1.f), fminf(fmaxf(t.w, -1.f), 1.f)};
  return t;
}

template <int LPR_LOG2, int HPB, int NEED, class C>
__device__ inline void long_row_chunk(const AggArgs& a, const FastRsrc& R, int c, int lane, float* lds_w,
                                      const float* lds_bias, const float* lds_scale) {
  constexpr int LPR = 1 << LPR_LOG2, G = 64 / LPR;
  const int g = lane >> LPR_LOG2;
  const int q = lane & (LPR - 1);
  const unsigned slot_off = (unsigned)q * 16u;
  const unsigned row_bytes = (unsigned)a.ldb * 4u;
  const bool lane_live = q < C::slots(a);
  const bool looped_any = C::xl(a) || C::yl(a);
  if (c >= a.plan[1]) return;
  const int cap_long = a.plan[2], cap_chunks = a.plan[3];
  const int* long_row = a.plan + 4;
  const int* long_chunk0 = long_row + cap_long;
  const int* chunk_slot = long_chunk0 + cap_long;
  const int* chunk_begin = chunk_slot + cap_chunks;
  const int slot = __builtin_amdgcn_readfirstlane(chunk_slot[c]);
  const int row = __builtin_amdgcn_readfirstlane(long_row[slot]);
  if (row < a.row_begin || row >= a.row_end) return;
  const int start = __builtin_amdgcn_readfirstlane(chunk_begin[c]);
  const int row_start = __builtin_amdgcn_readfirstlane(a.rowptr[row]);
  const int row_end = __builtin_amdgcn_readfirstlane(a.rowptr[row + 1]);
  const int end = min(start + EGC_LONG_ROW_CHUNK, row_end);
  const int deg = row_end - row_start;
  const int nch = (deg + EGC_LONG_ROW_CHUNK - 1) / EGC_LONG_ROW_CHUNK;
  const float dis_i = a.dis != nullptr ? a.dis[row] : 0.f;
  FAcc<NEED> acc;
  acc.init();
  f4 shift = f4{0.f, 0.f, 0.f, 0.f};
  if constexpr (NEED & NEED_SQ) {
    const int first = __builtin_amdgcn_readfirstlane(a.col[row_start]);
    shift = load_slot(R.bases, lane_live ? (unsigned)first * row_bytes + slot_off : OOB);
    acc.sh = shift;
  }
  int nself = 0;
  for (int base = start; base < end; base += 64) {
    const int p = base + lane;
    const bool pv = p < end;
    const int jj = pv ? a.col[p] : row;
    const float dd = a.edis != nullptr ? (pv ? a.edis[p] : 0.f) : (a.dis != nullptr ? a.dis[jj] : 0.f);
    if (looped_any) nself += __popcll(__ballot(pv && jj == row));
    const int cnt = min(64, end - base);
    for (int t0 = 0; t0 < cnt; t0 += FU * G)
      gather_batch<NEED, C>(a, R, acc, (g + t0) << 2, G << 2, row, jj, dd, dis_i, lane_live ? cnt : 0, t0 + g, G, row_bytes,
                            slot_off, base);
  }
  all_reduce_groups<LPR_LOG2, NEED>(acc, lane);
  if (nch > 1) {
    constexpr int WT = 0x11;
    constexpr int REC = (NEED & NEED_ARG) ? 7 : 5;
    const __amdgpu_buffer_rsrc_t pw = __builtin_amdgcn_make_buffer_rsrc(
        (void*)(reinterpret_cast<f4*>(a.partial) + (int64_t)c * REC * LPR), 0, (unsigned)REC * LPR * 16u, 0x00020000);
    const unsigned po = (g == 0 && lane_live) ? (unsigned)q * 16u : OOB;
    __builtin_amdgcn_raw_buffer_store_b128(__builtin_bit_cast(u32x4, acc.sum), pw, po, 0 * LPR * 16, WT);
    __builtin_amdgcn_raw_buffer_store_b128(__builtin_bit_cast(u32x4, acc.mx), pw, po, 2 * LPR * 16, WT);
    __builtin_amdgcn_raw_buffer_store_b128(__builtin_bit_cast(u32x4, acc.ws), pw, po, 4 * LPR * 16, WT);
    if constexpr (NEED & NEED_SQ)
      __builtin_amdgcn_raw_buffer_store_b128(__builtin_bit_cast(u32x4, acc.sq), pw, po, 1 * LPR * 16, WT);
    if constexpr (NEED & NEED_MN)
      __builtin_amdgcn_raw_buffer_store_b128(__builtin_bit_cast(u32x4, acc.mn), pw, po, 3 * LPR * 16, WT);
    if constexpr (NEED & NEED_ARG) {
      __builtin_amdgcn_raw_buffer_store_b128(__builtin_bit_cast(u32x4, acc.ax), pw, po, 5 * LPR * 16, WT);
      if constexpr (NEED & NEED_MN)
        __builtin_amdgcn_raw_buffer_store_b128(__builtin_bit_cast(u32x4, acc.an), pw, po, 6 * LPR * 16, WT);
    }
    const __amdgpu_buffer_rsrc_t pn =
        __builtin_amdgcn_make_buffer_rsrc((void*)(a.partial_nself + c), 0, 4u, 0x00020000);
    __builtin_amdgcn_raw_buffer_store_b32(nself, pn, lane == 0 ? 0u : OOB, 0, WT);
    asm volatile("s_waitcnt vmcnt(0)" ::: "memory");
    int arrived = 0;
    if (lane == 0) arrived = __hip_atomic_fetch_add(&a.counters[slot], 1, __ATOMIC_RELAXED, __HIP_MEMORY_SCOPE_AGENT);
    arrived = __builtin_amdgcn_readfirstlane(arrived);
    if (arrived != nch - 1) return;
    __builtin_amdgcn_fence(__ATOMIC_ACQUIRE, "agent");
    asm volatile("s_waitcnt vmcnt(0)" ::: "memory");
    if (lane == 0) __hip_atomic_store(&a.counters[slot], 0, __ATOMIC_RELAXED, __HIP_MEMORY_SCOPE_AGENT);
    const int c0 = __builtin_amdgcn_readfirstlane(long_chunk0[slot]);
    acc.init();
    if constexpr (NEED & NEED_SQ) acc.sh = shift;
    constexpr int MU = 4;
    const __amdgpu_buffer_rsrc_t prs = __builtin_amdgcn_make_buffer_rsrc(
        (void*)(reinterpret_cast<const f4*>(a.partial) + (int64_t)c0 * REC * LPR), 0,
        (unsigned)nch * (unsigned)REC * LPR * 16u, 0x00020000);
    for (int k0 = g; k0 < nch; k0 += G * MU) {
      f4 rs[MU], rm[MU], rw[MU], rq[MU], rn[MU], rax[MU], ran[MU];
  #pragma unroll
      for (int m = 0; m < MU; ++m) {
        const int kk = k0 + m * G;
        const unsigned off = (kk < nch && lane_live) ? ((unsigned)kk * (unsigned)REC * LPR + (unsigned)q) * 16u : OOB;
        rs[m] = load_slot_wt(prs, off);
        rm[m] = load_slot_wt(prs, off == OOB ? OOB : off + 2u * LPR * 16u);
        rw[m] = load_slot_wt(prs, off == OOB ? OOB : off + 4u * LPR * 16u);
        if constexpr (NEED & NEED_SQ) rq[m] = load_slot_wt(prs, off == OOB ? OOB : off + 1u * LPR * 16u);
        if constexpr (NEED & NEED_MN) rn[m] = load_slot_wt(prs, off == OOB ? OOB : off + 3u * LPR * 16u);
        if constexpr (NEED & NEED_ARG) {
          rax[m] = load_slot_wt(prs, off == OOB ? OOB : off + 5u * LPR * 16u);
          if constexpr (NEED & NEED_MN) ran[m] = load_slot_wt(prs, off == OOB ? OOB : off + 6u * LPR * 16u);
        }
      }
  #pragma unroll
      for (int m = 0; m < MU; ++m) {
        acc.sum += rs[m];
        acc.ws += rw[m];
        if constexpr (NEED & NEED_SQ) acc.sq += rq[m];
        if (k0 + m * G < nch) {
          if constexpr (NEED & NEED_ARG) {
            merge_gt4(acc.mx, acc.ax, rm[m], __builtin_bit_cast(i4, rax[m]));
            if constexpr (NEED & NEED_MN) merge_lt4(acc.mn, acc.an, rn[m], __builtin_bit_cast(i4, ran[m]));
          } else {
            acc.mx = f4_vmax(acc.mx, rm[m]);
            if constexpr (NEED & NEED_MN) acc.mn = f4_vmin(acc.mn, rn[m]);
          }
        }
      }
    }
    all_reduce_groups<LPR_LOG2, NEED>(acc, lane);
    nself = 0;
    for (int k = lane; k < nch; k += 64)
      nself += __hip_atomic_load(&a.partial_nself[c0 + k], __ATOMIC_RELAXED, __HIP_MEMORY_SCOPE_AGENT);
  #pragma unroll
    for (int off = 32; off > 0; off >>= 1) nself += bperm((lane ^ off) << 2, nself);
  }
  f4 wpre[2], vself;
// ... 8 lines not shown
```

egc_amd/csrc/egc_common.h:

```cpp
#pragma once
#include <hip/hip_runtime.h>
#include <stdint.h>

#include "egc_hip.h"
#include "egc_plain.h"

#define EGC_WAVE 64

namespace egc {

void set_last_error(const char* what, hipError_t err);

#define EGC_HIP_TRY(expr)                          \
  do {                                             \
    hipError_t _e = (expr);                        \
    if (_e != hipSuccess) {                        \
      ::egc::set_last_error(#expr, _e);            \
      return EGC_ERR_HIP;                          \
    }                                              \
  } while (0)

#define EGC_LAUNCH_CHECK(name)                     \
  do {                                             \
    hipError_t _e = hipGetLastError();             \
    if (_e != hipSuccess) {                        \
      ::egc::set_last_error(name, _e);             \
      return EGC_ERR_HIP;                          \
    }                                              \
  } while (0)

#define EGC_ALLOW_DYNAMIC_LDS(kernel, bytes, what)                                                              \
  do {                                                                                                          \
    static bool _allowed = false;                                                                               \
    if (!_allowed) {                                                                                            \
      hipError_t _e = hipFuncSetAttribute(reinterpret_cast<const void*>(kernel),                                \
                                          hipFuncAttributeMaxDynamicSharedMemorySize, (int)(bytes));            \
      if (_e != hipSuccess) {                                                                                   \
        ::egc::set_last_error("hipFuncSetAttribute(" what ")", _e);                                             \
        return EGC_ERR_HIP;                                                                                     \
      }                                                                                                         \
      _allowed = true;                                                                                          \
    }                                                                                                           \
  } while (0)

typedef float f32x16 __attribute__((ext_vector_type(16)));
typedef float f32x2 __attribute__((ext_vector_type(2)));
typedef float f4 __attribute__((ext_vector_type(4)));
typedef _Float16 f16x8 __attribute__((ext_vector_type(8)));
typedef _Float16 f16x2 __attribute__((ext_vector_type(2)));
typedef __bf16 bf16x8 __attribute__((ext_vector_type(8)));
typedef unsigned short u16;
typedef unsigned int u32x2 __attribute__((ext_vector_type(2)));
typedef unsigned int u32x4 __attribute__((ext_vector_type(4)));

__device__ inline void lds_barrier() { asm volatile("s_waitcnt lgkmcnt(0)\n\ts_barrier" ::: "memory"); }

template <bool VEC>
__device__ inline f4 tm_load(const float* __restrict__ p, int c, int width) {
  if (VEC) return *reinterpret_cast<const f4*>(p);
  f4 v = f4{0.f, 0.f, 0.f, 0.f};
#pragma unroll
  for (int j = 0; j < 4; ++j)
    if (c + j < width) v[j] = p[j];
  return v;
}

template <bool VEC>
__device__ inline void tm_store(float* __restrict__ p, int c, int width, f4 v) {
  if (VEC) {
    *reinterpret_cast<f4*>(p) = v;
    return;
  }
#pragma unroll
  for (int j = 0; j < 4; ++j)
    if (c + j < width) p[j] = v[j];
}

typedef int i4 __attribute__((ext_vector_type(4)));

template <bool VEC>
__device__ inline i4 tm_load_i(const int32_t* __restrict__ p, int c, int width) {
  if (VEC) return *reinterpret_cast<const i4*>(p);
  i4 v = i4{-1, -1, -1, -1};
#pragma unroll
  for (int j = 0; j < 4; ++j)
    if (c + j < width) v[j] = p[j];
  return v;
}

template <bool VEC>
__device__ inline void tm_store_i(int32_t* __restrict__ p, int c, int width, i4 v) {
  if (VEC) {
    *reinterpret_cast<i4*>(p) = v;
    return;
  }
#pragma unroll
  for (int j = 0; j < 4; ++j)
    if (c + j < width) p[j] = v[j];
}

static inline bool tm_aligned16(const void* p) { return (reinterpret_cast<uintptr_t>(p) & 15) == 0; }

int arg_extrema(const egc_graph* graph, const egc_layer* layer, const float* bases, int32_t ldb, const float* stats,
                const int32_t* cnt, int32_t* arg_max, int32_t* arg_min, unsigned* arg8_max, unsigned* arg8_min,
                hipStream_t stream);

int launch_segment_reduce(const float* x, const int64_t* seg_ptr, int64_t n_segments, int64_t n_rows, int32_t width,
                          int32_t op, float* out, int32_t* arg, hipStream_t stream);

}
```

egc_amd/csrc/egc_graph.hip:

```cpp
#include <algorithm>
#include <cstring>
#include <string>

#include <rocprim/device/device_radix_sort.hpp>
#include <rocprim/iterator/counting_iterator.hpp>

#include "egc_common.h"

namespace egc {

static thread_local std::string g_last_error;

void set_last_error(const char* what, hipError_t err) {
  g_last_error = std::string(what) + ": " + hipGetErrorString(err);
}


__global__ void __launch_bounds__(256) coo_keys_kernel(const int64_t* __restrict__ src,
                                                       const int64_t* __restrict__ dst, int64_t n_edges,
                                                       uint32_t* __restrict__ keys, int32_t* __restrict__ max_index,
                                                       int64_t n_nodes, int64_t n_src, int32_t* __restrict__ status,
                                                       int32_t* __restrict__ host_flag) {
  __shared__ int wave_max[4];
  int64_t e = (int64_t)blockIdx.x * blockDim.x + threadIdx.x;
  int m = -1;
  bool bad = false;
  for (; e < n_edges; e += (int64_t)gridDim.x * blockDim.x) {
    const int64_t s64 = src[e], d64 = dst[e];
    if (status != nullptr && (s64 < 0 || s64 >= n_src || d64 < 0 || d64 >= n_nodes)) {
      keys[e] = (uint32_t)n_nodes;
      bad = true;
      continue;
    }
    int s = (int)s64, d = (int)d64;
    keys[e] = (uint32_t)d;
    m = max(m, max(s, d));
  }
  if (__ballot(bad) != 0 && (threadIdx.x & 63) == 0) {
    atomicOr(status, 1);
    if (host_flag != nullptr) *(volatile int32_t*)host_flag = 1;
  }
#pragma unroll
  for (int off = 32; off > 0; off >>= 1) m = max(m, __shfl_xor(m, off));
  if ((threadIdx.x & 63) == 0) wave_max[threadIdx.x >> 6] = m;
  __syncthreads();
  if (threadIdx.x == 0) {
    m = max(max(wave_max[0], wave_max[1]), max(wave_max[2], wave_max[3]));
    if (m >= 0) atomicMax(max_index, m);
  }
}

__global__ void __launch_bounds__(256) gather_col_kernel(const int64_t* __restrict__ src,
                                                         const uint32_t* __restrict__ edge_id, int64_t n_edges,
                                                         int32_t* __restrict__ col, const int32_t* __restrict__ n_kept) {
  int64_t p = (int64_t)blockIdx.x * blockDim.x + threadIdx.x;
  const int64_t kept = n_kept != nullptr ? (int64_t)*n_kept : n_edges;
  for (; p < n_edges; p += (int64_t)gridDim.x * blockDim.x) col[p] = p < kept ? (int32_t)src[edge_id[p]] : 0;
}

__global__ void __launch_bounds__(256) rowptr_kernel(const uint32_t* __restrict__ sorted_dst, int64_t n_edges,
                                                     int64_t n_nodes, int32_t* __restrict__ rowptr) {
  int64_t i = (int64_t)blockIdx.x * blockDim.x + threadIdx.x;
  if (i > n_nodes) return;
  int64_t lo = 0, hi = n_edges;
  while (lo < hi) {
    int64_t mid = (lo + hi) >> 1;
    if ((int64_t)sorted_dst[mid] < i) lo = mid + 1; else hi = mid;
  }
  rowptr[i] = (int32_t)lo;
}

constexpr int PREP_ROWS = 64;
constexpr int PREP_HUGE = 2048;
__global__ void __launch_bounds__(16 * PREP_ROWS) prepare_kernel(int64_t n_nodes, const int32_t* __restrict__ rowptr,
                                                                 const int32_t* __restrict__ col,
                                                                 float* __restrict__ dis_raw, float* __restrict__ dis_looped,
                                                                 int32_t* __restrict__ plan, int cap_long, int cap_chunks) {
  __shared__ int s_long, s_chunks, s_base_long, s_base_chunk;
  __shared__ int s_huge_n, s_huge_row[PREP_ROWS], s_huge_cnt[PREP_ROWS];
  const int sl = threadIdx.x & 15;
  const int64_t row = (int64_t)blockIdx.x * PREP_ROWS + (threadIdx.x >> 4);
  const bool live = row < n_nodes;
  if (threadIdx.x == 0) { s_long = 0; s_chunks = 0; s_huge_n = 0; }
  __syncthreads();
  const int start = live ? rowptr[row] : 0, end = live ? rowptr[row + 1] : 0;
  const int deg = end - start;
  if (dis_looped != nullptr) {
    if (deg > PREP_HUGE) {
      if (sl == 0) {
        const int h = atomicAdd(&s_huge_n, 1);
        s_huge_row[h] = (int)(threadIdx.x >> 4);
        s_huge_cnt[h] = 0;
      }
    } else {
      int nonself = 0;
      for (int p = start + sl; p < end; p += 16) nonself += (col[p] != (int)row);
#pragma unroll
      for (int off = 8; off > 0; off >>= 1) nonself += __shfl_xor(nonself, off);
      if (live && sl == 0) dis_looped[row] = 1.0f / sqrtf((float)(nonself + 1));
    }
    __syncthreads();
    for (int h = 0; h < s_huge_n; ++h) {
      const int64_t hr = (int64_t)blockIdx.x * PREP_ROWS + s_huge_row[h];
      const int hs = rowptr[hr], he = rowptr[hr + 1];
      int nonself = 0;
      for (int p = hs + (int)threadIdx.x; p < he; p += 16 * PREP_ROWS) nonself += (col[p] != (int)hr);
#pragma unroll
      for (int off = 32; off > 0; off >>= 1) nonself += __shfl_xor(nonself, off);
      if ((threadIdx.x & 63) == 0 && nonself != 0) atomicAdd(&s_huge_cnt[h], nonself);
      __syncthreads();
      if (threadIdx.x == 0) dis_looped[hr] = 1.0f / sqrtf((float)(s_huge_cnt[h] + 1));
    }
  }
  if (live && sl == 0 && dis_raw != nullptr) dis_raw[row] = deg > 0 ? 1.0f / sqrtf((float)deg) : 0.0f;
  const bool is_long = live && deg > EGC_LONG_ROW_THRESHOLD;
  const int nch = is_long ? (deg + EGC_LONG_ROW_CHUNK - 1) / EGC_LONG_ROW_CHUNK : 0;
  int slot = 0, c0 = 0;
  if (is_long && sl == 0) {
    slot = atomicAdd(&s_long, 1);
    c0 = atomicAdd(&s_chunks, nch);
  }
  __syncthreads();
  if (threadIdx.x == 0 && s_long > 0) {
    s_base_long = atomicAdd(&plan[0], s_long);
    s_base_chunk = atomicAdd(&plan[1], s_chunks);
  }
  __syncthreads();
  if (is_long) {
    slot = __shfl(slot, threadIdx.x & 48) + s_base_long;
    c0 = __shfl(c0, threadIdx.x & 48) + s_base_chunk;
    int32_t* long_row = plan + 4;
    int32_t* long_chunk0 = long_row + cap_long;
    int32_t* chunk_slot = long_chunk0 + cap_long;
    int32_t* chunk_begin = chunk_slot + cap_chunks;
    if (slot < cap_long && c0 + nch <= cap_chunks) {
      if (sl == 0) {
        long_row[slot] = (int32_t)row;
        long_chunk0[slot] = c0;
      }
      for (int k = sl; k < nch; k += 16) {
        chunk_slot[c0 + k] = slot;
        chunk_begin[c0 + k] = start + k * EGC_LONG_ROW_CHUNK;
      }
    }
  }
}

__global__ void __launch_bounds__(256) edge_dis_kernel(int64_t n_edges, const int32_t* __restrict__ col,
                                                       const float* __restrict__ dis_raw, const float* __restrict__ dis_looped,
                                                       float* __restrict__ out_raw, float* __restrict__ out_looped) {
  int64_t p = (int64_t)blockIdx.x * blockDim.x + threadIdx.x;
  for (; p < n_edges; p += (int64_t)gridDim.x * blockDim.x) {
    const int j = col[p];
    if (out_raw != nullptr) out_raw[p] = dis_raw[j];
    if (out_looped != nullptr) out_looped[p] = dis_looped[j];
  }
}

__global__ void __launch_bounds__(256) csr_transposed_coo_kernel(int n_nodes, int64_t n_edges, const int32_t* __restrict__ rowptr,
                                                                 const int32_t* __restrict__ col, int64_t* __restrict__ out_src,
                                                                 int64_t* __restrict__ out_dst) {
  int64_t p = (int64_t)blockIdx.x * blockDim.x + threadIdx.x;
  const int64_t kept = rowptr[n_nodes];
  for (; p < n_edges; p += (int64_t)gridDim.x * blockDim.x) {
    if (p >= kept) {
      out_src[p] = -1;
      out_dst[p] = -1;
      continue;
    }
    int lo = 0, hi = n_nodes;
    while (hi - lo > 1) {
      const int mid = (lo + hi) >> 1;
      if ((int64_t)rowptr[mid] <= p) lo = mid; else hi = mid;
    }
    out_src[p] = lo;
    out_dst[p] = col[p];
  }
}


constexpr int BUILD_SCAN_ITEMS = 4096;
constexpr int BUILD_LDS_SORT = 4096;
constexpr int BUILD_WAVE_ROW = BUILD_LDS_SORT / 16;
constexpr int BUILD_RANK_ROW = 1024;

constexpr int BUILD_TILE = 2048;
constexpr int BUILD_WIN = 2048;

struct TileEdges {
  int s[8], d[8];
  int dmin, dmax;
  bool bad;
};

__device__ inline TileEdges load_tile(const int64_t* __restrict__ src, const int64_t* __restrict__ dst, int64_t n_edges,
                                      int n_nodes, int n_src, int* s_min, int* s_max) {
  TileEdges t;
  t.bad = false;
  int lo = 0x7fffffff, hi = -1;
#pragma unroll
  for (int k = 0; k < 8; ++k) {
    const int64_t e = (int64_t)blockIdx.x * BUILD_TILE + k * 256 + threadIdx.x;
    t.s[k] = t.d[k] = -1;
    if (e < n_edges) {
      const int64_t s = src[e], d = dst[e];
      if (s < 0 || s >= n_src || d < 0 || d >= n_nodes) { t.bad = true; continue; }
      t.s[k] = (int)s;
      t.d[k] = (int)d;
      lo = min(lo, (int)d);
      hi = max(hi, (int)d);
    }
  }
  if (threadIdx.x == 0) { *s_min = 0x7fffffff; *s_max = -1; }
  __syncthreads();
#pragma unroll
  for (int off = 32; off > 0; off >>= 1) { lo = min(lo, __shfl_xor(lo, off)); hi = max(hi, __shfl_xor(hi, off)); }
  if ((threadIdx.x & 63) == 0) { atomicMin(s_min, lo); atomicMax(s_max, hi); }
  __syncthreads();
  t.dmin = *s_min;
  t.dmax = *s_max;
  return t;
}

__global__ void __launch_bounds__(256) build_hist_kernel(const int64_t* __restrict__ src, const int64_t* __restrict__ dst,
                                                         int64_t n_edges, int n_nodes, int n_src, int* __restrict__ deg,
                                                         int* __restrict__ deg_ns, int* __restrict__ maxp1,
                                                         int* __restrict__ status, int32_t* __restrict__ plan,
                                                         int cap_long, int cap_chunks, int32_t* __restrict__ host_flag) {
  __shared__ int s_cnt[BUILD_WIN], s_ns[BUILD_WIN];
  __shared__ int s_min, s_max, s_top;
  if (blockIdx.x == 0 && threadIdx.x == 0) {
    plan[0] = 0; plan[1] = 0; plan[2] = cap_long; plan[3] = cap_chunks;
  }
  const TileEdges t = load_tile(src, dst, n_edges, n_nodes, n_src, &s_min, &s_max);
  if (__ballot(t.bad) != 0 && (threadIdx.x & 63) == 0) {
    atomicOr(status, 1);
    if (host_flag != nullptr) *(volatile int32_t*)host_flag = 1;
  }
  if (t.dmin > t.dmax) return;
  int m = 0;
#pragma unroll
// ... 13 lines not shown
    __syncthreads();
    for (int w = threadIdx.x; w < span; w += 256) {
      const int c = s_cnt[w], cn = s_ns[w];
      if (c) atomicAdd(&deg[t.dmin + w], c);
      if (cn) atomicAdd(&deg_ns[t.dmin + w], cn);
    }
  } else {
    __syncthreads();
#pragma unroll
    for (int k = 0; k < 8; ++k)
      if (t.d[k] >= 0) {
        atomicAdd(&deg[t.d[k]], 1);
        if (t.s[k] != t.d[k]) atomicAdd(&deg_ns[t.d[k]], 1);
      }
  }
#pragma unroll
  for (int off = 32; off > 0; off >>= 1) m = max(m, __shfl_xor(m, off));
  if ((threadIdx.x & 63) == 0) atomicMax(&s_top, m);
  __syncthreads();
  if (threadIdx.x == 0 && s_top > 0) atomicMax(maxp1, s_top);
}

__global__ void __launch_bounds__(1024) build_sums_kernel(const int* __restrict__ deg, int n_nodes, int* __restrict__ bsum) {
  __shared__ int ws[16];
  const int base = blockIdx.x * BUILD_SCAN_ITEMS + threadIdx.x * 4;
  int v = 0;
#pragma unroll
  for (int k = 0; k < 4; ++k) v += (base + k < n_nodes) ? deg[base + k] : 0;
#pragma unroll
  for (int off = 32; off > 0; off >>= 1) v += __shfl_xor(v, off);
  if ((threadIdx.x & 63) == 0) ws[threadIdx.x >> 6] = v;
  __syncthreads();
  if (threadIdx.x == 0) {
    int t = 0;
    for (int k = 0; k < 16; ++k) t += ws[k];
    bsum[blockIdx.x] = t;
  }
}

__global__ void __launch_bounds__(1024) build_scan_kernel(const int* __restrict__ deg, int* __restrict__ deg_ns, int n_nodes,
                                                          int* __restrict__ bsum, int n_blocks, int* __restrict__ rowptr,
                                                          float* __restrict__ dis_raw, float* __restrict__ dis_looped,
                                                          int* __restrict__ maxp1, int32_t* __restrict__ max_index,
                                                          int32_t* __restrict__ plan, int cap_long, int cap_chunks) {
  __shared__ int ws[16];
  __shared__ int s_prefix;
  int p = 0;
  for (int k = threadIdx.x; k < (int)blockIdx.x; k += 1024) p += bsum[k];
#pragma unroll
  for (int off = 32; off > 0; off >>= 1) p += __shfl_xor(p, off);
  if ((threadIdx.x & 63) == 0) ws[threadIdx.x >> 6] = p;
  __syncthreads();
  if (threadIdx.x == 0) {
    int t = 0;
    for (int k = 0; k < 16; ++k) t += ws[k];
    s_prefix = t;
  }
  __syncthreads();
  const int base = blockIdx.x * BUILD_SCAN_ITEMS + threadIdx.x * 4;
  int d[4], dn[4];
#pragma unroll
  for (int k = 0; k < 4; ++k) {
    const bool ok = base + k < n_nodes;
    d[k] = ok ? deg[base + k] : 0;
    dn[k] = ok ? deg_ns[base + k] : 0;
  }
  int mine = d[0] + d[1] + d[2] + d[3];
  int incl = mine;
#pragma unroll
  for (int off = 1; off < 64; off <<= 1) {
    const int t = __shfl_up(incl, off);
    if ((int)(threadIdx.x & 63) >= off) incl += t;
  }
  __syncthreads();
  if ((threadIdx.x & 63) == 63) ws[threadIdx.x >> 6] = incl;
  __syncthreads();
  int wave_off = 0;
  for (int k = 0; k < (int)(threadIdx.x >> 6); ++k) wave_off += ws[k];
  int run = s_prefix + wave_off + incl - mine;
#pragma unroll
  for (int k = 0; k < 4; ++k) {
    if (base + k < n_nodes) {
      rowptr[base + k] = run;
      if (dis_raw != nullptr) dis_raw[base + k] = d[k] > 0 ? 1.0f / sqrtf((float)d[k]) : 0.0f;
      if (dis_looped != nullptr) dis_looped[base + k] = 1.0f / sqrtf((float)(dn[k] + 1));
      deg_ns[base + k] = 0;
      if (d[k] > EGC_LONG_ROW_THRESHOLD) {
        const int slot = atomicAdd(&plan[0], 1);
        const int c0 = atomicAdd(&plan[1], (d[k] + EGC_LONG_ROW_CHUNK - 1) / EGC_LONG_ROW_CHUNK);
        if (slot < cap_long) { plan[4 + slot] = base + k; plan[4 + cap_long + slot] = c0; }
      }
    }
    run += d[k];
  }
  if (base <= n_nodes && n_nodes < base + 4) rowptr[n_nodes] = run - 0;
  __syncthreads();
  if (blockIdx.x == (unsigned)n_blocks - 1 && threadIdx.x == 0) {
    *max_index = *maxp1 - 1;
    *maxp1 = 0;
  }
}

__global__ void __launch_bounds__(256) build_scatter_kernel(const int64_t* __restrict__ src, const int64_t* __restrict__ dst,
                                                            int64_t n_edges, int n_nodes, int n_src, int* __restrict__ deg,
                                                            const int* __restrict__ rowptr, int* __restrict__ col,
                                                            int* __restrict__ edge_id, int* __restrict__ bsum, int n_blocks) {
  __shared__ int s_cnt[BUILD_WIN], s_base[BUILD_WIN];
  __shared__ int s_min, s_max;
  if (blockIdx.x == 0)
    for (int k = threadIdx.x; k < n_blocks; k += blockDim.x) bsum[k] = 0;
  const TileEdges t = load_tile(src, dst, n_edges, n_nodes, n_src, &s_min, &s_max);
  if (t.dmin > t.dmax) return;
  const int span = t.dmax - t.dmin + 1;
  if (span <= BUILD_WIN) {
    for (int w = threadIdx.x; w < span; w += 256) s_cnt[w] = 0;
    __syncthreads();
#pragma unroll
    for (int k = 0; k < 8; ++k)
      if (t.d[k] >= 0) atomicAdd(&s_cnt[t.d[k] - t.dmin], 1);
    __syncthreads();
    for (int w = threadIdx.x; w < span; w += 256) {
      const int c = s_cnt[w];
      if (c) s_base[w] = rowptr[t.dmin + w] + atomicSub(&deg[t.dmin + w], c) - c;
      s_cnt[w] = 0;
    }
    __syncthreads();
#pragma unroll
    for (int k = 0; k < 8; ++k)
      if (t.d[k] >= 0) {
        const int w = t.d[k] - t.dmin;
        const int pos = s_base[w] + atomicAdd(&s_cnt[w], 1);
        col[pos] = t.s[k];
        edge_id[pos] = (int)((int64_t)blockIdx.x * BUILD_TILE + k * 256 + threadIdx.x);
      }
  } else {
#pragma unroll
    for (int k = 0; k < 8; ++k)
      if (t.d[k] >= 0) {
        const int pos = rowptr[t.d[k]] + atomicSub(&deg[t.d[k]], 1) - 1;
        col[pos] = t.s[k];
        edge_id[pos] = (int)((int64_t)blockIdx.x * BUILD_TILE + k * 256 + threadIdx.x);
      }
  }
}

__device__ inline void bitonic_steps(int2* kv, int n, int base, int k, int j_first) {
  for (int j = j_first; j > 0; j >>= 1) {
    for (int t = threadIdx.x; t < n; t += blockDim.x) {
      const int l = t ^ j;
      if (l > t) {
        const int2 a = kv[t], b = kv[l];
        const bool up = ((base + t) & k) == 0;
        if ((a.x > b.x) == up) { kv[t] = b; kv[l] = a; }
      }
    }
    __syncthreads();
  }
}

__device__ inline void bitonic_big(int2* g, int np2, int2* lds) {
  constexpr int C = BUILD_LDS_SORT;
  for (int c0 = 0; c0 < np2; c0 += C) {
    for (int t = threadIdx.x; t < C; t += blockDim.x) lds[t] = g[c0 + t];
    __syncthreads();
    for (int k = 2; k <= C; k <<= 1) bitonic_steps(lds, C, c0, k, k >> 1);
    for (int t = threadIdx.x; t < C; t += blockDim.x) g[c0 + t] = lds[t];
    __syncthreads();
  }
// ... 260 lines not shown
extern "C" {

const char* egc_last_error(void) { return g_last_error.c_str(); }

const char* egc_version(void) { return "egc_hip 0.3.0 gfx950"; }

int64_t egc_plan_ints(int64_t n_nodes, int64_t n_edges) {
  if (n_nodes < 0 || n_edges < 0) return -1;
  PlanCaps c = plan_caps(n_nodes, n_edges);
  return 4 + 2 * c.cap_long + 2 * c.cap_chunks;
}

size_t egc_coo_to_csr_workspace_bytes(int64_t n_nodes, int64_t n_edges) {
  if (n_nodes < 0 || n_edges < 0) return 0;
  size_t temp = 0;
  if (sort_temp_bytes(n_nodes + 1, n_edges, &temp) != hipSuccess) return 0;
  return 2 * align256((size_t)n_edges * sizeof(uint32_t)) + align256(temp) + 256;
}

int egc_coo_to_csr(const int64_t* src, const int64_t* dst, int64_t n_edges, int64_t n_nodes, int32_t* rowptr,
                   int32_t* col, int32_t* edge_id, int32_t* max_index, void* workspace, size_t workspace_bytes,
                   egc_stream_t stream_) {
  return egc_coo_to_csr_checked(src, dst, n_edges, n_nodes, 0, rowptr, col, edge_id, max_index, nullptr, nullptr, workspace,
                                workspace_bytes, stream_);
}

int egc_coo_to_csr_checked(const int64_t* src, const int64_t* dst, int64_t n_edges, int64_t n_nodes, int64_t n_src_rows,
                           int32_t* rowptr, int32_t* col, int32_t* edge_id, int32_t* max_index, int32_t* status,
                           int32_t* host_flag, void* workspace, size_t workspace_bytes, egc_stream_t stream_) {
  hipStream_t stream = (hipStream_t)stream_;
  if (n_nodes < 0 || n_edges < 0 || n_nodes >= ((int64_t)1 << 31) - 1 || n_edges >= ((int64_t)1 << 31) - 1)
    return EGC_ERR_INVALID;
  if (rowptr == nullptr || max_index == nullptr) return EGC_ERR_INVALID;
  if (n_edges > 0 && (src == nullptr || dst == nullptr || col == nullptr || edge_id == nullptr)) return EGC_ERR_INVALID;

  init_scalar_kernel<<<1, 1, 0, stream>>>(max_index, -1);
  EGC_LAUNCH_CHECK("init_scalar_kernel");
  if (status != nullptr) {
    init_scalar_kernel<<<1, 1, 0, stream>>>(status, 0);
    EGC_LAUNCH_CHECK("init_scalar_kernel");
  }
  if (n_edges == 0) {
    EGC_HIP_TRY(hipMemsetAsync(rowptr, 0, (size_t)(n_nodes + 1) * sizeof(int32_t), stream));
    return EGC_OK;
  }
  const int64_t n_src = n_src_rows > 0 ? n_src_rows : n_nodes;
  const int64_t n_keys = status != nullptr ? n_nodes + 1 : n_nodes;
  size_t temp = 0;
  EGC_HIP_TRY(sort_temp_bytes(n_keys, n_edges, &temp));
  const size_t kbytes = align256((size_t)n_edges * sizeof(uint32_t));
  if (workspace == nullptr || workspace_bytes < 2 * kbytes + align256(temp)) return EGC_ERR_WORKSPACE;
  char* ws = (char*)workspace;
  uint32_t* keys_in = (uint32_t*)ws;
  uint32_t* keys_out = (uint32_t*)(ws + kbytes);
  void* sort_temp = ws + 2 * kbytes;

  const int threads = 256;
  const int blocks = (int)std::min<int64_t>(ceil_div(n_edges, threads), 256 * 8);
  const int key_blocks = std::min(blocks, 512);
  coo_keys_kernel<<<key_blocks, threads, 0, stream>>>(src, dst, n_edges, keys_in, max_index, n_nodes, n_src, status, host_flag);
  EGC_LAUNCH_CHECK("coo_keys_kernel");
  EGC_HIP_TRY(rocprim::radix_sort_pairs(sort_temp, temp, (const uint32_t*)keys_in, keys_out,
                                        rocprim::counting_iterator<uint32_t>(0), (uint32_t*)edge_id,
                                        (size_t)n_edges, 0u, key_bits(n_keys), stream));
  rowptr_kernel<<<(int)ceil_div(n_nodes + 1, threads), threads, 0, stream>>>(keys_out, n_edges, n_nodes, rowptr);
  EGC_LAUNCH_CHECK("rowptr_kernel");
  gather_col_kernel<<<blocks, threads, 0, stream>>>(src, (const uint32_t*)edge_id, n_edges, col,
                                                    status != nullptr ? rowptr + n_nodes : nullptr);
  EGC_LAUNCH_CHECK("gather_col_kernel");
  return EGC_OK;
}

int egc_csr_edge_dis(int64_t n_edges, const int32_t* col, const float* dis_raw, const float* dis_looped,
                     float* edge_dis_raw, float* edge_dis_looped, egc_stream_t stream_) {
  hipStream_t stream = (hipStream_t)stream_;
  if (n_edges < 0) return EGC_ERR_INVALID;
  if (dis_raw == nullptr) edge_dis_raw = nullptr;
  if (dis_looped == nullptr) edge_dis_looped = nullptr;
  if (n_edges == 0 || (edge_dis_raw == nullptr && edge_dis_looped == nullptr)) return EGC_OK;
  if (col == nullptr) return EGC_ERR_INVALID;
  const int blocks = (int)std::min<int64_t>(ceil_div(n_edges, 256), 256 * 8);
  edge_dis_kernel<<<blocks, 256, 0, stream>>>(n_edges, col, dis_raw, dis_looped, edge_dis_raw, edge_dis_looped);
  EGC_LAUNCH_CHECK("edge_dis_kernel");
  return EGC_OK;
}

int egc_csr_transposed_coo(int64_t n_nodes, int64_t n_edges, const int32_t* rowptr, const int32_t* col, int64_t* out_src,
                           int64_t* out_dst, egc_stream_t stream_) {
  hipStream_t stream = (hipStream_t)stream_;
  if (n_nodes < 0 || n_edges < 0 || n_nodes >= (1ll << 31) || n_edges >= (1ll << 31)) return EGC_ERR_INVALID;
  if (n_edges == 0) return EGC_OK;
  if (n_nodes == 0 || rowptr == nullptr || col == nullptr || out_src == nullptr || out_dst == nullptr) return EGC_ERR_INVALID;
  const unsigned blocks = (unsigned)std::min<int64_t>(ceil_div(n_edges, (int64_t)256), 8192);
  csr_transposed_coo_kernel<<<blocks, 256, 0, stream>>>((int)n_nodes, n_edges, rowptr, col, out_src, out_dst);
  EGC_LAUNCH_CHECK("csr_transposed_coo_kernel");
  return EGC_OK;
}

int egc_gather_rows_f32(const float* table, int64_t ld, const int64_t* idx, int64_t n_rows, int32_t width, float* out,
                        egc_stream_t stream_) {
  hipStream_t stream = (hipStream_t)stream_;
  if (n_rows < 0 || width <= 0 || (width & 3) != 0 || (ld & 3) != 0 || ld < width) return EGC_ERR_INVALID;
  if (n_rows == 0) return EGC_OK;
  if (table == nullptr || idx == nullptr || out == nullptr) return EGC_ERR_INVALID;
  if (((uintptr_t)table & 15) != 0 || ((uintptr_t)out & 15) != 0) return EGC_ERR_INVALID;
  const int64_t pieces = n_rows * (width / 4);
  const unsigned blocks = (unsigned)std::min<int64_t>(ceil_div(pieces, (int64_t)256), 256 * 16);
  gather_rows_kernel<<<blocks, 256, 0, stream>>>((const float4*)table, idx, pieces, width / 4, ld / 4, (float4*)out);
  EGC_LAUNCH_CHECK("gather_rows_kernel");
  return EGC_OK;
}

size_t egc_graph_build_workspace_bytes(int64_t n_nodes, int64_t n_edges) {
  if (n_nodes < 0 || n_edges < 0) return 0;
  const int64_t nb = ceil_div(n_nodes + 1, (int64_t)BUILD_SCAN_ITEMS);
  return align256((size_t)(n_nodes + 1) * 4) + align256((size_t)n_nodes * 4 + 4) + align256((size_t)nb * 4) + 256;
}

size_t egc_graph_build_scratch_bytes(int64_t n_edges) {
  if (n_edges < 0) return 0;
  return align256((size_t)n_edges * 2 * sizeof(int2)) + 256;
}

int egc_graph_build(const int64_t* src, const int64_t* dst, int64_t n_edges, int64_t n_nodes, int64_t n_src_rows,
                    int32_t* rowptr, int32_t* col, int32_t* edge_id, int32_t* max_index, float* dis_raw,
                    float* dis_looped, float* edge_dis_raw, float* edge_dis_looped, int32_t* plan, int32_t* status,
                    int32_t* host_flag, void* workspace, size_t workspace_bytes, void* scratch, size_t scratch_bytes,
                    egc_stream_t stream_) {
  hipStream_t stream = (hipStream_t)stream_;
  if (n_nodes < 0 || n_edges < 0 || n_nodes >= ((int64_t)1 << 30) || n_edges >= ((int64_t)1 << 30)) return EGC_ERR_INVALID;
  if (rowptr == nullptr || max_index == nullptr || plan == nullptr || status == nullptr) return EGC_ERR_INVALID;
  if (n_edges > 0 && (src == nullptr || dst == nullptr || col == nullptr || edge_id == nullptr)) return EGC_ERR_INVALID;
  if (workspace == nullptr || workspace_bytes < egc_graph_build_workspace_bytes(n_nodes, n_edges)) return EGC_ERR_WORKSPACE;
  if (scratch == nullptr || scratch_bytes < egc_graph_build_scratch_bytes(n_edges)) return EGC_ERR_WORKSPACE;
  if (dis_raw == nullptr) edge_dis_raw = nullptr;
  if (dis_looped == nullptr) edge_dis_looped = nullptr;
  const int64_t n_src = n_src_rows > 0 ? n_src_rows : n_nodes;
  const int nb = (int)ceil_div(n_nodes + 1, (int64_t)BUILD_SCAN_ITEMS);
  char* ws = (char*)workspace;
  int* deg = (int*)ws;
  int* deg_ns = (int*)(ws + align256((size_t)(n_nodes + 1) * 4));
  int* bsum = (int*)((char*)deg_ns + align256((size_t)n_nodes * 4 + 4));
  int* maxp1 = (int*)((char*)bsum + align256((size_t)nb * 4));
  int* ws_status = maxp1 + 1;
  int2* big = (int2*)scratch;
  PlanCaps c = plan_caps(n_nodes, n_edges);
  if (n_nodes == 0) {
    plan_header_kernel<<<1, 1, 0, stream>>>(plan, (int)c.cap_long, (int)c.cap_chunks);
    init_scalar_kernel<<<1, 1, 0, stream>>>(status, n_edges > 0 ? 1 : 0);
    if (n_edges > 0 && host_flag != nullptr) init_scalar_kernel<<<1, 1, 0, stream>>>(host_flag, 1);
    init_scalar_kernel<<<1, 1, 0, stream>>>(max_index, -1);
    EGC_HIP_TRY(hipMemsetAsync(rowptr, 0, sizeof(int32_t), stream));
    EGC_LAUNCH_CHECK("egc_graph_build(empty)");
    return EGC_OK;
  }
  const int eblocks = (int)std::max<int64_t>(1, ceil_div(n_edges, (int64_t)BUILD_TILE));
  build_hist_kernel<<<eblocks, 256, 0, stream>>>(src, dst, n_edges, (int)n_nodes, (int)n_src, deg, deg_ns, maxp1, ws_status, plan,
                                             (int)c.cap_long, (int)c.cap_chunks, host_flag);
  EGC_LAUNCH_CHECK("build_hist_kernel");
  build_sums_kernel<<<nb, 1024, 0, stream>>>(deg, (int)n_nodes, bsum);
  EGC_LAUNCH_CHECK("build_sums_kernel");
  build_scan_kernel<<<nb, 1024, 0, stream>>>(deg, deg_ns, (int)n_nodes, bsum, nb, rowptr, dis_raw, dis_looped, maxp1, max_index, plan,
                                             (int)c.cap_long, (int)c.cap_chunks);
  EGC_LAUNCH_CHECK("build_scan_kernel");
  build_scatter_kernel<<<eblocks, 256, 0, stream>>>(src, dst, n_edges, (int)n_nodes, (int)n_src, deg, rowptr, col, edge_id, bsum, nb);
  EGC_LAUNCH_CHECK("build_scatter_kernel");
// ... 24 lines not shown
```

egc_amd/graph.py:

```python
from __future__ import annotations

import ctypes as C
import os
from collections import OrderedDict

import torch

from . import _C


def _stream_ptr(device) -> int:
    idx = device.index if isinstance(device, torch.device) else device
    if idx is None:
        idx = torch.cuda.current_device()
    return torch._C._cuda_getCurrentRawStream(idx)


class _NoGuard:
    def __enter__(self):
        return self

    def __exit__(self, *exc):
        return False


_NO_GUARD = _NoGuard()


def _device_guard(device):
    idx = device.index if isinstance(device, torch.device) else device
    if idx is None or idx == torch.cuda.current_device():
        return _NO_GUARD
    return torch.cuda.device(device)


class _IndexFlag:
    _word = None
    _view = None

    @classmethod
    def ptr(cls) -> int:
        if cls._word is None:
            cls._word = torch.zeros(1, dtype=torch.int32).pin_memory()
            cls._view = C.c_int32.from_address(cls._word.data_ptr())
        return cls._word.data_ptr()

    @classmethod
    def poll(cls):
        if cls._view is not None and cls._view.value != 0:
            cls._view.value = 0
            raise RuntimeError("egc_amd: an earlier call reported malformed graph input: an edge_index with node ids outside "
                               "[0, num_nodes): index out of range (those edges were dropped) -- or, for a GraphBatch, edges that "
                               "leave their graph / a graph larger than max_nodes (its rows were written as zeros; "
                               "GraphBatch.check() tells which) -- or, for a node encoder, an index outside its embedding table (that "
                               "table contributed a zero row)")


def _require_cuda(t: torch.Tensor, what: str):
    if not t.is_cuda:
        raise RuntimeError(
            f"egc_amd: {what} must live on a ROCm device (got {t.device}); the EGC hot path is HIP-only "
            "and has no CPU fallback")


class CSRGraph:

    def __init__(self, n_nodes, n_edges, rowptr, col, edge_id, dis_raw, dis_looped, max_index, plan, n_src_rows=None):
        self.n_nodes, self.n_edges = int(n_nodes), int(n_edges)
        self.n_src_rows = int(n_src_rows) if n_src_rows is not None else int(n_nodes)
        self.halo = None
        self.rowptr, self.col, self.edge_id = rowptr, col, edge_id
        self.dis_raw, self.dis_looped, self.max_index, self.plan = dis_raw, dis_looped, max_index, plan
        self.device = rowptr.device
        self.edge_dis_raw = self.edge_dis_looped = None
        self._workspaces = {}
        self._n_chunks = None

    @classmethod
    def from_edge_index(cls, edge_index: torch.Tensor, num_nodes: int, num_src_rows: int | None = None,
                        build: str = "auto", _poll: bool = True) -> "CSRGraph":
        _require_cuda(edge_index, "edge_index")
        if edge_index.dtype != torch.int64 or edge_index.dim() != 2 or edge_index.size(0) != 2:
            raise RuntimeError("egc_amd: edge_index must be an int64 tensor of shape [2, E]")
        if _poll:
            _IndexFlag.poll()
        lib = _C.load()
        dev = edge_index.device
        ei = edge_index.contiguous()
        n, e = int(num_nodes), int(ei.size(1))
        build = os.environ.get("EGC_GRAPH_BUILD", build)
        if build not in ("auto", "fast", "sort"):
            raise RuntimeError(f"egc_amd: build must be 'auto', 'fast' or 'sort', got {build!r}")
        if build == "auto":
            build = "fast" if (e <= _FAST_BUILD_SMALL or (e <= _FAST_BUILD_MAX_EDGES and e <= 10 * n)) else "sort"
        if build == "fast" and e <= _FAST_BUILD_MAX_EDGES:
            return cls._build_fast(ei, n, e, num_src_rows)
        with _device_guard(dev):
            e1 = max(e, 1)
            plan_ints = int(lib.egc_plan_ints(n, e))
            sizes = (n + 1, e1, e1, 1, plan_ints, 1)
            offs, total = [], 0
            for sz in sizes:
                offs.append(total)
                total += (sz + 3) & ~3
            slab = torch.empty(total, dtype=torch.int32, device=dev)
            rowptr, col, edge_id, max_index, plan, status = (slab[o:o + sz] for o, sz in zip(offs, sizes))
            ws_bytes = lib.egc_coo_to_csr_workspace_bytes(n, e)
            ws = torch.empty(max(ws_bytes, 1), dtype=torch.uint8, device=dev)
            _C.check(lib.egc_coo_to_csr_checked(ei[0].data_ptr(), ei[1].data_ptr(), e, n,
                                                int(num_src_rows) if num_src_rows is not None else 0, rowptr.data_ptr(),
                                                col.data_ptr(), edge_id.data_ptr(), max_index.data_ptr(), status.data_ptr(),
                                                _IndexFlag.ptr(), ws.data_ptr(), ws.numel(), _stream_ptr(dev)),
                     "egc_coo_to_csr_checked")
            g = cls._prepare(n, e, rowptr, col, edge_id, max_index, num_src_rows, plan=plan)
            g._status = status
            if os.environ.get("EGC_CHECK_INDICES", "0") not in ("", "0"):
                g.check_indices()
            return g

    @classmethod
    def _build_fast(cls, ei: torch.Tensor, n: int, e: int, num_src_rows) -> "CSRGraph":
        lib = _C.load()
        dev = ei.device
        ns = n if num_src_rows is None else int(num_src_rows)
        if ns <= 0 and e > 0:
            raise RuntimeError("egc_amd: num_src_rows must be positive")
        square = ns == n
        with _device_guard(dev):
            e1 = max(e, 1)
            plan_ints = int(lib.egc_plan_ints(n, e))
            sizes = (n + 1, e1, e1, 1, plan_ints, 1)
            offs, total = [], 0
            for sz in sizes:
                offs.append(total)
                total += (sz + 3) & ~3
            slab = torch.empty(total, dtype=torch.int32, device=dev)
            rowptr, col, edge_id, max_index, plan, status = (slab[o:o + sz] for o, sz in zip(offs, sizes))
            nrow = max(n, ns, 1)
            nd, ee = (nrow + 3) & ~3, (e1 + 3) & ~3
            fslab = torch.empty(2 * nd + (2 * ee if square else 0), dtype=torch.float32, device=dev)
            dis_raw, dis_looped = fslab[:nrow], fslab[nd:nd + nrow]
            if nrow > n:
                fslab[:2 * nd].zero_()
            edr = fslab[2 * nd:2 * nd + e1] if square else None
            edl = fslab[2 * nd + ee:2 * nd + ee + e1] if square else None
            ws = _build_workspace(dev, int(lib.egc_graph_build_workspace_bytes(n, e)))
            scratch = torch.empty(int(lib.egc_graph_build_scratch_bytes(e)), dtype=torch.uint8, device=dev)
            _C.check(lib.egc_graph_build(ei[0].data_ptr(), ei[1].data_ptr(), e, n, ns, rowptr.data_ptr(), col.data_ptr(),
                                         edge_id.data_ptr(), max_index.data_ptr(), dis_raw.data_ptr(), dis_looped.data_ptr(),
                                         edr.data_ptr() if edr is not None else None,
                                         edl.data_ptr() if edl is not None else None, plan.data_ptr(), status.data_ptr(),
                                         _IndexFlag.ptr(), ws.data_ptr(), ws.numel(), scratch.data_ptr(), scratch.numel(),
                                         _stream_ptr(dev)),
                     "egc_graph_build")
        g = cls(n, e, rowptr, col, edge_id, dis_raw, dis_looped, max_index, plan, ns)
        g.edge_dis_raw, g.edge_dis_looped = edr, edl
        g._status = status
        if os.environ.get("EGC_CHECK_INDICES", "0") not in ("", "0"):
            g.check_indices()
        return g

    def check_indices(self) -> "CSRGraph":
        st = getattr(self, "_status", None)
        if st is not None and int(st.item()) != 0:
            if _IndexFlag._view is not None:
                _IndexFlag._view.value = 0
            raise RuntimeError("egc_amd: edge_index holds node ids outside [0, num_nodes): index out of range")
        return self

    @classmethod
    def from_partition(cls, edge_index_local: torch.Tensor, plan, global_max_index: int | None = None,
                       exchange_dis: bool = True) -> "CSRGraph":
        g = cls.from_edge_index(edge_index_local, plan.n_local, plan.n_local + plan.n_halo)
        g.halo = plan
        if global_max_index is not None:
            if plan.order is not None and int(global_max_index) < plan.n_global - 1:
                raise RuntimeError("egc_amd: interior_first partitions need global_max_index == n_global - 1 "
                                   "(trailing isolated vertices: build the partition with interior_first=False)")
            g.max_index.fill_(max(-1, min(int(global_max_index) - plan.lo, plan.n_local - 1)))
        if exchange_dis and plan.n_halo >= 0 and plan.world > 1:
            plan.exchange(g.dis_raw)
            plan.exchange(g.dis_looped)
            g.refresh_edge_dis()
        return g

    @classmethod
    def from_csr(cls, rowptr: torch.Tensor, col: torch.Tensor, num_nodes: int | None = None,
                 num_src_rows: int | None = None) -> "CSRGraph":
        _require_cuda(rowptr, "rowptr")
        dev = rowptr.device
        n = int(rowptr.numel() - 1) if num_nodes is None else int(num_nodes)
        e = int(col.numel())
        rowptr = rowptr.to(torch.int32).contiguous()
        col32 = col.to(torch.int32).contiguous() if e > 0 else torch.empty(1, dtype=torch.int32, device=dev)
        with _device_guard(dev):
            edge_id = torch.arange(max(e, 1), dtype=torch.int32, device=dev)
            max_index = torch.full((1,), n - 1, dtype=torch.int32, device=dev)
            return cls._prepare(n, e, rowptr, col32, edge_id, max_index, num_src_rows)

    @classmethod
    def _prepare(cls, n, e, rowptr, col, edge_id, max_index, n_src_rows=None, plan=None) -> "CSRGraph":
        lib = _C.load()
        dev = rowptr.device
        ns = n if n_src_rows is None else int(n_src_rows)
        if ns <= 0 and e > 0:
            raise RuntimeError("egc_amd: num_src_rows must be positive")
        nd, e1 = (max(n, ns, 1) + 3) & ~3, (max(e, 1) + 3) & ~3
        square = ns == n
        fslab = torch.empty(2 * nd + (2 * e1 if square else 0), dtype=torch.float32, device=dev)
        dis_raw, dis_looped = fslab[:max(n, ns, 1)], fslab[nd:nd + max(n, ns, 1)]
        if max(n, ns, 1) > n:
            fslab[:2 * nd].zero_()
        if plan is None:
            plan = torch.empty(lib.egc_plan_ints(n, e), dtype=torch.int32, device=dev)
        _C.check(lib.egc_csr_prepare(n, e, rowptr.data_ptr(), col.data_ptr(), dis_raw.data_ptr(),
                                     dis_looped.data_ptr(), plan.data_ptr(), _stream_ptr(dev)), "egc_csr_prepare")
        g = cls(n, e, rowptr, col, edge_id, dis_raw, dis_looped, max_index, plan, ns)
        if square:
            g.edge_dis_raw = fslab[2 * nd:2 * nd + max(e, 1)]
            g.edge_dis_looped = fslab[2 * nd + e1:2 * nd + e1 + max(e, 1)]
            g.refresh_edge_dis()
        return g

    def refresh_edge_dis(self):
        lib = _C.load()
        dev = self.device
        e = self.n_edges
        with _device_guard(dev):
            if self.edge_dis_raw is None:
                self.edge_dis_raw = torch.empty(max(e, 1), dtype=torch.float32, device=dev)
                self.edge_dis_looped = torch.empty(max(e, 1), dtype=torch.float32, device=dev)
            _C.check(lib.egc_csr_edge_dis(e, self.col.data_ptr(), self.dis_raw.data_ptr(), self.dis_looped.data_ptr(),
                                          self.edge_dis_raw.data_ptr(), self.edge_dis_looped.data_ptr(),
                                          _stream_ptr(dev)), "egc_csr_edge_dis")

    def transposed(self) -> "CSRGraph":
        if getattr(self, "_transposed", None) is None:
            dev = self.device
            n, e, ns = self.n_nodes, self.n_edges, self.n_src_rows
            with _device_guard(dev):
                coo = torch.empty((2, e), dtype=torch.int64, device=dev)
                _C.check(_C.load().egc_csr_transposed_coo(n, e, self.rowptr.data_ptr(), self.col.data_ptr(),
                                                          coo[0].data_ptr(), coo[1].data_ptr() if e else None,
                                                          _stream_ptr(dev)), "egc_csr_transposed_coo")
                self._transposed = CSRGraph.from_edge_index(coo, ns, max(n, 1), _poll=False)
        if self._n_chunks is not None and self._n_chunks >= 0:
            self._transposed.trim_launches()
        return self._transposed

    def workspace(self, nbytes: int, zero_bytes: int | None = None) -> torch.Tensor:
        key = (int(nbytes), _stream_ptr(self.device))
        ws = self._workspaces.get(key)
        if ws is None:
            n = max(int(nbytes), 1)
            if zero_bytes is None or zero_bytes >= n:
                ws = torch.zeros(n, dtype=torch.uint8, device=self.device)
            else:
                ws = torch.empty(n, dtype=torch.uint8, device=self.device)
                ws[:int(zero_bytes)].zero_()
            self._workspaces[key] = ws
        return ws

    def c_struct(self) -> _C.EgcGraph:
        _IndexFlag.poll()
        if self._n_chunks is None:
            self._n_chunks = -1
        return _C.EgcGraph(self.n_nodes, self.n_edges, self.rowptr.data_ptr(), self.col.data_ptr(),
                           self.edge_id.data_ptr(), self.dis_raw.data_ptr(), self.dis_looped.data_ptr(),
                           self.max_index.data_ptr(), self.plan.data_ptr(), self._n_chunks, self.n_src_rows,
                           self.edge_dis_raw.data_ptr() if self.edge_dis_raw is not None else None,
                           self.edge_dis_looped.data_ptr() if self.edge_dis_looped is not None else None)

    def tensors(self) -> list:
        ts = [self.rowptr, self.col, self.edge_id, self.dis_raw, self.dis_looped, self.max_index, self.plan]
        return ts + [t for t in (self.edge_dis_raw, self.edge_dis_looped) if t is not None]

    def c_addr(self) -> int:
        key = (self._n_chunks, 0 if self.edge_dis_raw is None else self.edge_dis_raw.data_ptr(),
               0 if self.edge_dis_looped is None else self.edge_dis_looped.data_ptr())
        hit = getattr(self, "_c_cached", None)
        if hit is None or hit[0] != key or self._n_chunks is None:
            st = self.c_struct()
            key = (self._n_chunks, key[1], key[2])
            hit = self._c_cached = (key, st, C.addressof(st))
        else:
            _IndexFlag.poll()
        return hit[2]

    def workspace_for(self, spec) -> torch.Tensor:
        cache = self.__dict__.setdefault("_ws_for", {})
        key = (id(spec), _stream_ptr(self.device), self._n_chunks)
        ws = cache.get(key)
        if ws is None:
            lib = _C.load()
            g = self.c_struct()
            ws = self.workspace(lib.egc_aggregate_workspace_bytes_for(C.byref(spec.c), C.byref(g)),
                                lib.egc_aggregate_workspace_zero_bytes(C.byref(spec.c), self.n_nodes, self.n_edges))
            cache[(id(spec), _stream_ptr(self.device), self._n_chunks)] = ws
            cache.setdefault("_keep", []).append(spec)
        return ws

    def trim_launches(self) -> "CSRGraph":
        if self._n_chunks is None or self._n_chunks < 0:
            self._n_chunks = int(self.plan[1].item())
            self.check_indices()
        return self

    def long_row_stats(self):
        h = self.plan[:2].cpu()
        return int(h[0]), int(h[1])


_FAST_BUILD_MAX_EDGES = 4_000_000
_FAST_BUILD_SMALL = 262_144
_BUILD_WS: "dict[tuple, torch.Tensor]" = {}


def _build_workspace(dev, nbytes: int) -> torch.Tensor:
    if torch.cuda.is_current_stream_capturing():
        return torch.zeros(max(int(nbytes), 1 << 12), dtype=torch.uint8, device=dev)
    key = (str(dev), _stream_ptr(dev))
    ws = _BUILD_WS.get(key)
    if ws is None or ws.numel() < nbytes:
        ws = torch.zeros(max(int(nbytes * 1.25), 1 << 20), dtype=torch.uint8, device=dev)
        _BUILD_WS[key] = ws
    return ws


def drop_stream_workspaces(stream) -> None:
    raw = stream.cuda_stream
    for key in [k for k in _BUILD_WS if k[1] == raw]:
        del _BUILD_WS[key]


class SparseTensor:

    def __init__(self, row: torch.Tensor = None, col: torch.Tensor = None, value=None, sparse_sizes=None,
                 is_sorted: bool = False, rowptr: torch.Tensor = None):
        if sparse_sizes is None:
            raise RuntimeError("egc_amd.SparseTensor: sparse_sizes=(N_dst, N_src) is required")
        self._sizes = (int(sparse_sizes[0]), int(sparse_sizes[1]))
        if rowptr is not None:
            self.graph = CSRGraph.from_csr(rowptr, col, self._sizes[0], self._sizes[1])
        else:
            self.graph = CSRGraph.from_edge_index(torch.stack([col.long(), row.long()]), self._sizes[0], self._sizes[1])
        self.graph.trim_launches()

    def sparse_sizes(self):
        return self._sizes

    def sparse_size(self, dim):
        return self._sizes[dim]

    def size(self, dim):
        return self._sizes[dim]


_TILE_SETUPS: "dict[tuple, object]" = {}


_STATUS_POOLS: dict = {}


def _status_word(device: torch.device) -> torch.Tensor:
    key = (device.type, device.index)
    pool = _STATUS_POOLS.get(key)
    if pool is None or pool[1] >= pool[0].numel():
        pool = [torch.zeros(1024, dtype=torch.int32, device=device), 0]
        _STATUS_POOLS[key] = pool
    i = pool[1]
    pool[1] = i + 1
    return pool[0][i:i + 1]


class GraphBatch:

    def __init__(self, edge_index: torch.Tensor, ptr: torch.Tensor | None = None, batch: torch.Tensor | None = None,
                 num_graphs: int | None = None, num_nodes: int | None = None, max_nodes: int = 256, edges_per_node: int = 16,
                 edge_ptr: torch.Tensor | None = None):
        _require_cuda(edge_index, "edge_index")
        if edge_index.dtype != torch.int64 or edge_index.dim() != 2 or edge_index.size(0) != 2:
            raise RuntimeError("egc_amd: edge_index must be an int64 tensor of shape [2, E]")
        self.edge_index = edge_index.contiguous()
        self.device = edge_index.device
        if ptr is None:
            if batch is None or num_graphs is None:
                raise RuntimeError("egc_amd.GraphBatch: pass ptr (node offsets of the graphs, int64 [G + 1]) or batch "
                                   "together with num_graphs")
# ... 248 lines not shown
```

include/egc_hip.h:

```cpp
#ifndef EGC_HIP_H
#define EGC_HIP_H

#include <stddef.h>
#include <stdint.h>

#ifdef __cplusplus
extern "C" {
#endif

typedef void* egc_stream_t;

typedef enum {
  EGC_OK = 0,
  EGC_ERR_INVALID = 1,
  EGC_ERR_WORKSPACE = 2,
  EGC_ERR_HIP = 3,
  EGC_ERR_UNSUPPORTED = 4
} egc_status;

typedef enum {
  EGC_AGGR_SUM = 0, EGC_AGGR_MEAN = 1, EGC_AGGR_MAX = 2, EGC_AGGR_MIN = 3,
  EGC_AGGR_VAR = 4, EGC_AGGR_STD = 5, EGC_AGGR_SYMNORM = 6
} egc_aggr;

typedef enum { EGC_SET_RAW = 0, EGC_SET_LOOPED = 1 } egc_edge_set;

typedef enum { EGC_LAYOUT_HBA = 0, EGC_LAYOUT_HAB = 1 } egc_weight_layout;

typedef enum { EGC_ACT_NONE = 0, EGC_ACT_SOFTMAX = 1, EGC_ACT_SIGMOID = 2, EGC_ACT_HARDTANH = 3 } egc_weight_act;

#define EGC_MAX_AGGRS 8
#define EGC_MAX_BASIS_WIDTH 1024
#define EGC_MAX_WEIGHT_WIDTH 2048
#define EGC_MAX_OUT_CHANNELS 2048

#define EGC_LONG_ROW_THRESHOLD 64
#define EGC_LONG_ROW_CHUNK 256

typedef struct {
  int64_t n_nodes;
  int64_t n_edges;
  const int32_t* rowptr;
  const int32_t* col;
  const int32_t* edge_id;
  const float* dis_raw;
  const float* dis_looped;
  const int32_t* max_index;
  const int32_t* plan;
  int64_t n_chunks;
  int64_t n_src_rows;
  const float* edge_dis_raw;
  const float* edge_dis_looped;
} egc_graph;

int64_t egc_plan_ints(int64_t n_nodes, int64_t n_edges);

size_t egc_coo_to_csr_workspace_bytes(int64_t n_nodes, int64_t n_edges);

int egc_coo_to_csr(const int64_t* src, const int64_t* dst, int64_t n_edges, int64_t n_nodes,
                   int32_t* rowptr, int32_t* col, int32_t* edge_id, int32_t* max_index,
                   void* workspace, size_t workspace_bytes, egc_stream_t stream);

int egc_coo_to_csr_checked(const int64_t* src, const int64_t* dst, int64_t n_edges, int64_t n_nodes, int64_t n_src_rows,
                           int32_t* rowptr, int32_t* col, int32_t* edge_id, int32_t* max_index, int32_t* status,
                           int32_t* host_flag, void* workspace, size_t workspace_bytes, egc_stream_t stream);

size_t egc_graph_build_workspace_bytes(int64_t n_nodes, int64_t n_edges);
size_t egc_graph_build_scratch_bytes(int64_t n_edges);
int egc_graph_build(const int64_t* src, const int64_t* dst, int64_t n_edges, int64_t n_nodes, int64_t n_src_rows,
                    int32_t* rowptr, int32_t* col, int32_t* edge_id, int32_t* max_index, float* dis_raw,
                    float* dis_looped, float* edge_dis_raw, float* edge_dis_looped, int32_t* plan, int32_t* status,
                    int32_t* host_flag, void* workspace, size_t workspace_bytes, void* scratch, size_t scratch_bytes,
                    egc_stream_t stream);

int egc_csr_prepare(int64_t n_nodes, int64_t n_edges, const int32_t* rowptr, const int32_t* col,
                    float* dis_raw, float* dis_looped, int32_t* plan, egc_stream_t stream);

int egc_csr_transposed_coo(int64_t n_nodes, int64_t n_edges, const int32_t* rowptr, const int32_t* col, int64_t* out_src,
                           int64_t* out_dst, egc_stream_t stream);

int egc_csr_edge_dis(int64_t n_edges, const int32_t* col, const float* dis_raw, const float* dis_looped,
                     float* edge_dis_raw, float* edge_dis_looped, egc_stream_t stream);

int egc_gather_rows_f32(const float* table, int64_t ld, const int64_t* idx, int64_t n_rows, int32_t width, float* out,
                        egc_stream_t stream);

typedef struct {
  int32_t in_channels;
  int32_t out_channels;
  int32_t num_heads;
  int32_t num_bases;
  int32_t num_aggrs;
  int32_t aggrs[EGC_MAX_AGGRS];
  int32_t agg_set;
  int32_t sym_set;
  int32_t loops_all_nodes;
  int32_t weight_layout;
  int32_t weight_act;
  int32_t basis_stride;
} egc_layer;

int32_t egc_bases_ld(const egc_layer* layer);

int egc_basis_transform_f32(const float* x, const float* wcat, const float* bcat, int64_t n_nodes,
                            int32_t f_in, int32_t f_g, int32_t w_cols, float* bases, int32_t ldb,
                            float* weightings, egc_stream_t stream);

size_t egc_basis_pack_bytes(int32_t f_in, int32_t f_g, int32_t w_cols);
int egc_basis_pack(const float* wcat, int32_t f_in, int32_t f_g, int32_t w_cols, void* packed,
                   size_t packed_bytes, egc_stream_t stream);
#define EGC_GEMM_24BIT 1
int32_t egc_layer_gemm_flags(const egc_layer* layer);
int egc_basis_pack_ex(const float* wcat, int32_t f_in, int32_t f_g, int32_t w_cols, int32_t flags, void* packed,
                      size_t packed_bytes, egc_stream_t stream);
int egc_basis_transform_packed_ex(const float* x, const void* packed, const float* bcat, int64_t n_nodes, int32_t f_in,
                                  int32_t f_g, int32_t w_cols, int32_t flags, float* bases, int32_t ldb,
                                  float* weightings, egc_stream_t stream);
int egc_basis_pack_transposed(const float* wt, int64_t ld, int32_t f_in, int32_t f_g, int32_t w_cols, void* packed,
                              size_t packed_bytes, egc_stream_t stream);
int egc_basis_transform_packed(const float* x, const void* packed, const float* bcat, int64_t n_nodes,
                               int32_t f_in, int32_t f_g, int32_t w_cols, float* bases, int32_t ldb,
                               float* weightings, egc_stream_t stream);
int egc_basis_transform_packed_add(const float* x, const void* packed, const float* bcat, int64_t n_nodes, int32_t f_in,
                                   int32_t f_g, int32_t w_cols, int32_t flags, const float* bases_addend, float* bases, int32_t ldb,
                                   float* weightings, egc_stream_t stream);

size_t egc_aggregate_workspace_bytes(const egc_layer* layer, int64_t n_nodes, int64_t n_edges);
size_t egc_aggregate_workspace_zero_bytes(const egc_layer* layer, int64_t n_nodes, int64_t n_edges);
size_t egc_aggregate_workspace_bytes_for(const egc_layer* layer, const egc_graph* graph);

int egc_aggregate_combine_f32(const egc_graph* graph, const egc_layer* layer, const float* bases, int32_t ldb,
                              const float* weightings, const float* bias, float* out,
                              int32_t* arg_max, int32_t* arg_min,
                              void* workspace, size_t workspace_bytes, egc_stream_t stream);

int egc_aggregate_combine_rows_f32(const egc_graph* graph, const egc_layer* layer, const float* bases, int32_t ldb,
                                   const float* weightings, const float* bias, float* out, int64_t row_begin,
                                   int64_t row_end, void* workspace, size_t workspace_bytes, egc_stream_t stream);

typedef struct {
  const float* scale;
  const float* shift;
  const float* residual;
  int32_t relu;
} egc_post;
int egc_aggregate_combine_post_f32(const egc_graph* graph, const egc_layer* layer, const float* bases, int32_t ldb,
                                   const float* weightings, const float* bias, const egc_post* post, float* out,
                                   void* workspace, size_t workspace_bytes, egc_stream_t stream);

int egc_aggregate_combine_strided_f32(const egc_graph* graph, const egc_layer* layer, const float* bases, int32_t ldb,
                                      const float* weightings, int32_t ldw, const float* bias, const egc_post* post,
                                      float* out, void* workspace, size_t workspace_bytes, egc_stream_t stream);

int64_t egc_weight_grad_workspace_bytes(int64_t n_rows, int32_t f_in, int32_t k_cols);
int egc_weight_grad_plan(int64_t n_rows, int32_t f_in, int32_t k_cols, int32_t* plan8);
int64_t egc_weight_grad_ex_workspace_bytes(int64_t n_rows, int32_t f_in, int32_t k_cols, int32_t e_cols);
int egc_weight_grad_ex_f32(const float* x, int64_t ldx, const float* d, int64_t ldd, int64_t n_rows, int32_t f_in,
                           int32_t k_cols, float* out, float* col_sums, const float* e, int64_t lde, int32_t e_cols,
                           float* e_sums, void* workspace, int64_t workspace_bytes, void* stream);
int egc_weight_grad_params_f32(const float* x, int64_t ldx, const float* d, int64_t ldd, int64_t n_rows, int32_t f_in,
                               int32_t num_heads, int32_t num_aggrs, int32_t num_bases, int32_t basis_len, int32_t basis_stride,
                               int32_t permute_hab, float* const* d_bases_parts, int32_t n_parts, float* d_comb_weight,
                               float* d_comb_bias, float* d_bcat, const float* e, int64_t lde, int32_t e_cols, float* e_sums,
                               void* workspace, int64_t workspace_bytes, void* stream);
int egc_weight_grad_f32(const float* x, int64_t ldx, const float* d, int64_t ldd, int64_t n_rows, int32_t f_in,
// ... 291 lines not shown
```

Baseline: 18.38 billion edges/s.

## Pack column index and symnorm degree count into one 32-bit edge word

Adds per-edge packed entries that store the source column in the low bits and the integer degree count behind the symnorm coefficient in the high bits. The aggregation kernel then rebuilds the coefficient with 1/sqrt(count) instead of loading a separate per-edge float. This targets the per-edge index and coefficient traffic. Entries whose float value cannot be reproduced bit-exactly fall back to the old edge_dis load through an escape path. The packed path is a separate template used only for the H=8, B=4 sum/mean/max/symnorm fast configuration. The packed arrays are built once when launches are trimmed.

```diff
diff --git a/egc_amd/_C.py b/egc_amd/_C.py
--- a/egc_amd/_C.py
+++ b/egc_amd/_C.py
@@ -36,6 +36,7 @@
         ("dis_raw", C.c_void_p), ("dis_looped", C.c_void_p),
         ("max_index", C.c_void_p), ("plan", C.c_void_p), ("n_chunks", C.c_int64),
         ("n_src_rows", C.c_int64), ("edge_dis_raw", C.c_void_p), ("edge_dis_looped", C.c_void_p),
+        ("entry_raw", C.c_void_p), ("entry_looped", C.c_void_p), ("entry_col_bits", C.c_int32),
     ]
 
 
@@ -81,6 +82,10 @@
                                   C.c_void_p, C.c_void_p, C.c_void_p, C.c_void_p, C.c_void_p, C.c_void_p, C.c_void_p,
                                   C.c_void_p, C.c_void_p, C.c_size_t, C.c_void_p, C.c_size_t, C.c_void_p]),
     "egc_csr_edge_dis": (C.c_int, [C.c_int64, C.c_void_p, C.c_void_p, C.c_void_p, C.c_void_p, C.c_void_p, C.c_void_p]),
+    "egc_entry_col_bits": (C.c_int32, [C.c_int64]),
+    "egc_csr_pack_entries": (C.c_int, [C.c_int64, C.c_void_p, C.c_void_p, C.c_void_p, C.c_int32, C.c_void_p, C.c_void_p,
+                                       C.c_void_p]),
+    "egc_csr_pack_entries_host": (C.c_int, [C.c_int64, C.c_void_p, C.c_void_p, C.c_void_p, C.c_int32, C.c_void_p, C.c_void_p]),
     "egc_csr_prepare": (C.c_int, [C.c_int64, C.c_int64, C.c_void_p, C.c_void_p, C.c_void_p, C.c_void_p,
                                   C.c_void_p, C.c_void_p]),
     "egc_bases_ld": (C.c_int32, [C.POINTER(EgcLayer)]),
diff --git a/egc_amd/csrc/egc_aggregate.hip b/egc_amd/csrc/egc_aggregate.hip
--- a/egc_amd/csrc/egc_aggregate.hip
+++ b/egc_amd/csrc/egc_aggregate.hip
@@ -608,6 +608,13 @@
     a.edis = layer->sym_set == EGC_SET_LOOPED ? graph->edge_dis_looped : graph->edge_dis_raw;
     if (a.dis == nullptr) return EGC_ERR_INVALID;
   }
+  a.entry = nullptr;
+  a.entry_bits = 0;
+  if (a.edis != nullptr && stats == nullptr && graph->entry_col_bits > 0 && graph->entry_col_bits <= 30 &&
+      getenv("EGC_NO_PACKED_ENTRIES") == nullptr) {
+    a.entry = reinterpret_cast<const unsigned*>(layer->sym_set == EGC_SET_LOOPED ? graph->entry_looped : graph->entry_raw);
+    a.entry_bits = a.entry != nullptr ? graph->entry_col_bits : 0;
+  }
   a.max_index = graph->max_index;
   if (layer->loops_all_nodes == 0 && graph->max_index == nullptr) return EGC_ERR_INVALID;
   a.plan = graph->plan;
diff --git a/egc_amd/csrc/egc_aggregate_dev.h b/egc_amd/csrc/egc_aggregate_dev.h
--- a/egc_amd/csrc/egc_aggregate_dev.h
+++ b/egc_amd/csrc/egc_aggregate_dev.h
@@ -46,6 +46,8 @@
   const int* col;
   const float* dis;
   const float* edis;
+  const unsigned* entry;
+  int entry_bits;
   const int* max_index;
   const int* plan;
   const float* bases;
@@ -131,8 +133,9 @@
   return f4{__shfl_xor(v.x, off), __shfl_xor(v.y, off), __shfl_xor(v.z, off), __shfl_xor(v.w, off)};
 }
 
+template <int AUX = 0>
 __device__ inline f4 load_slot(__amdgpu_buffer_rsrc_t rsrc, unsigned byte_off) {
-  return __builtin_bit_cast(f4, __builtin_amdgcn_raw_buffer_load_b128(rsrc, byte_off, 0, 0));
+  return __builtin_bit_cast(f4, __builtin_amdgcn_raw_buffer_load_b128(rsrc, byte_off, 0, AUX));
 }
 
 __device__ inline void fold(f4& sum, f4& sq, f4& mx, f4& mn, f4& ws, f4 v, bool in_x, bool in_y, float w, f4 sh) {
diff --git a/egc_amd/csrc/egc_aggregate_fast.hip b/egc_amd/csrc/egc_aggregate_fast.hip
--- a/egc_amd/csrc/egc_aggregate_fast.hip
+++ b/egc_amd/csrc/egc_aggregate_fast.hip
@@ -4,7 +4,7 @@
 
 namespace egc {
 
-template <int LPR_LOG2, int HPB, int NEED, class C>
+template <int LPR_LOG2, int HPB, int NEED, class C, bool PK = false>
 #ifndef EGC_AGG_WAVES_SQ
 #define EGC_AGG_WAVES_SQ 5
 #endif
@@ -47,7 +47,7 @@
 
   if ((int)blockIdx.x < a.chunk_blocks) {
     const int c = __builtin_amdgcn_readfirstlane(blockIdx.x * 4 + wave);
-    long_row_chunk<LPR_LOG2, HPB, NEED, C>(a, R, c, lane, lds_w, lds_bias, lds_scale);
+    long_row_chunk<LPR_LOG2, HPB, NEED, C, PK>(a, R, c, lane, lds_w, lds_bias, lds_scale);
     return;
   }
 
@@ -64,7 +64,8 @@
     const int deg = bperm((g + 1) << 2, rp) - start_n;
     nd_n = (r0 + g < n_end && deg <= EGC_LONG_ROW_THRESHOLD) ? deg : 0;
   }
-  int jj_n = q < nd_n ? a.col[start_n + q] : 0;
+  const int* stage = PK ? reinterpret_cast<const int*>(a.entry) : a.col;
+  int jj_n = q < nd_n ? stage[start_n + q] : 0;
   for (int k = 0; k < Q; ++k) {
     const int rbase = r0 + k * G;
     if (rbase >= n_end) break;
@@ -76,7 +77,7 @@
       start_n = bperm(((k + 1) * G + g) << 2, rp);
       const int deg = bperm(((k + 1) * G + g + 1) << 2, rp) - start_n;
       nd_n = (rbase + G + g < n_end && deg <= EGC_LONG_ROW_THRESHOLD) ? deg : 0;
-      jj_n = q < nd_n ? a.col[start_n + q] : 0;
+      jj_n = q < nd_n ? stage[start_n + q] : 0;
     }
     int maxd = nd;
 #pragma unroll
@@ -90,14 +91,21 @@
     FAcc<NEED> acc;
     acc.init();
     if constexpr (NEED & NEED_SQ) {
-      const int first = bperm(grp_addr, jj);
+      int first = bperm(grp_addr, jj);
+      if constexpr (PK) first = entry_col((unsigned)first, a.entry_bits);
       acc.sh = load_slot(R.bases, (lane_live && nd > 0) ? (unsigned)first * row_bytes + slot_off : OOB);
     }
     int nself = 0;
     for (int ts = 0; ts < maxd; ts += LPR) {
-      if (ts > 0) jj = (ts + q < nd) ? a.col[start + ts + q] : 0;
+      if (ts > 0) jj = (ts + q < nd) ? stage[start + ts + q] : 0;
       const bool pv = ts + q < nd;
-      const float dd = !pv ? 0.f : a.edis != nullptr ? a.edis[start + ts + q] : a.dis != nullptr ? a.dis[jj] : 0.f;
+      float dd;
+      if constexpr (PK) {
+        const unsigned word = (unsigned)jj;
+        entry_split(a, word, pv, start + ts + q, jj, dd);
+      } else {
+        dd = !pv ? 0.f : a.edis != nullptr ? a.edis[start + ts + q] : a.dis != nullptr ? a.dis[jj] : 0.f;
+      }
       if (looped_any) {
         const unsigned long long sb = __ballot(pv && jj == row);
         nself += __popcll((sb >> (g << LPR_LOG2)) & ((LPR == 64) ? ~0ull : ((1ull << LPR) - 1ull)));
@@ -436,20 +444,34 @@
   return true;
 }
 
-template <int LPR_LOG2, int HPB, int NEED, class C>
+template <int LPR_LOG2, int HPB, int NEED, class C, bool PK = false>
 static int launch_one(const AggArgs& a, unsigned grid, size_t lds, hipStream_t stream) {
-  agg_fast_kernel<LPR_LOG2, HPB, NEED, C><<<grid, 256, lds, stream>>>(a);
+  agg_fast_kernel<LPR_LOG2, HPB, NEED, C, PK><<<grid, 256, lds, stream>>>(a);
   EGC_LAUNCH_CHECK("agg_fast_kernel");
   return EGC_OK;
 }
 
+template <class C>
+constexpr bool cfg_reads_packed_entries() {
+  constexpr int S = EGC_AGGR_SUM, M = EGC_AGGR_MEAN, X = EGC_AGGR_MAX, Y = EGC_AGGR_SYMNORM;
+  return C::kH == 8 && C::kB == 4 && C::kL == 16 && C::kAct == EGC_ACT_NONE && C::kXl && C::kYl && C::kLoopsAll &&
+         (C::kAgg == agg_pack(S, M, X, Y) || C::kAgg == agg_pack(S, X, Y));
+}
+
 template <class C, int NEED>
 static bool try_static(const AggArgs& a, unsigned grid, size_t lds, hipStream_t stream, int* status) {
+  constexpr bool PK = NEED == 0 && cfg_reads_packed_entries<C>();
   constexpr int LPR_LOG2 = agg_lpr_log2(C::kB * C::P_), HPB = (C::kH + C::kB - 1) / C::kB;
   if (!cfg_matches<C>(a) || a.slots > (1 << LPR_LOG2) || 2 * a.slots <= (1 << LPR_LOG2)) return false;
   if constexpr (C::has(EGC_AGGR_MAX)) {
     if (a.arg_max != nullptr) {
       *status = launch_one<LPR_LOG2, HPB, NEED | NEED_ARG, C>(a, grid, lds, stream);
+      return true;
+    }
+  }
+  if constexpr (PK) {
+    if (a.entry != nullptr) {
+      *status = launch_one<LPR_LOG2, HPB, NEED, C, true>(a, grid, lds, stream);
       return true;
     }
   }
diff --git a/egc_amd/csrc/egc_aggregate_fast_dev.h b/egc_amd/csrc/egc_aggregate_fast_dev.h
--- a/egc_amd/csrc/egc_aggregate_fast_dev.h
+++ b/egc_amd/csrc/egc_aggregate_fast_dev.h
@@ -283,7 +283,17 @@
   __amdgpu_buffer_rsrc_t bases, out, res;
 };
 
-template <int NEED, class C>
+__device__ inline void entry_split(const AggArgs& a, unsigned word, bool pv, int p, int& jj, float& dd) {
+  jj = entry_col(word, a.entry_bits);
+  const int c = entry_count(word, a.entry_bits);
+  dd = (pv && c != 0) ? inv_sqrt_count(max(c, 1)) : 0.f;
+  const bool esc = pv && c == 0;
+  if (__ballot(esc) != 0) {
+    if (esc) dd = a.edis[p];
+  }
+}
+
+template <int NEED, class C, int AUX = 0>
 __device__ inline void gather_batch(const AggArgs& a, const FastRsrc& R, FAcc<NEED>& acc, int addr0, int step, int row,
                                     int jj, float dd, float dis_i, int n_valid, int first, int vstep,
                                     unsigned row_bytes, unsigned slot_off, int pos_base) {
@@ -296,7 +306,7 @@
     const int j = bperm(addr, jj);
     const bool is_self = j == row;
     in_x[u] = (first + u * vstep < n_valid) && !(C::xl(a) && is_self);
-    v[u] = load_slot(R.bases, in_x[u] ? (unsigned)j * row_bytes + slot_off : OOB);
+    v[u] = load_slot<AUX>(R.bases, in_x[u] ? (unsigned)j * row_bytes + slot_off : OOB);
     w[u] = bperm(addr, dd) * dis_i;
     if (C::yl(a) && !C::xl(a)) w[u] = is_self ? 0.f : w[u];
   }
@@ -562,7 +572,7 @@
   return t;
 }
 
-template <int LPR_LOG2, int HPB, int NEED, class C>
+template <int LPR_LOG2, int HPB, int NEED, class C, bool PK = false>
 __device__ inline void long_row_chunk(const AggArgs& a, const FastRsrc& R, int c, int lane, float* lds_w,
                                       const float* lds_bias, const float* lds_scale) {
   constexpr int LPR = 1 << LPR_LOG2, G = 64 / LPR;
@@ -600,8 +610,15 @@
   for (int base = start; base < end; base += 64) {
     const int p = base + lane;
     const bool pv = p < end;
-    const int jj = pv ? a.col[p] : row;
-    const float dd = a.edis != nullptr ? (pv ? a.edis[p] : 0.f) : (a.dis != nullptr ? a.dis[jj] : 0.f);
+    int jj;
+    float dd;
+    if constexpr (PK) {
+      entry_split(a, pv ? a.entry[p] : 0u, pv, p, jj, dd);
+      jj = pv ? jj : row;
+    } else {
+      jj = pv ? a.col[p] : row;
+      dd = a.edis != nullptr ? (pv ? a.edis[p] : 0.f) : (a.dis != nullptr ? a.dis[jj] : 0.f);
+    }
     if (looped_any) nself += __popcll(__ballot(pv && jj == row));
     const int cnt = min(64, end - base);
     for (int t0 = 0; t0 < cnt; t0 += FU * G)
diff --git a/egc_amd/csrc/egc_common.h b/egc_amd/csrc/egc_common.h
--- a/egc_amd/csrc/egc_common.h
+++ b/egc_amd/csrc/egc_common.h
@@ -52,6 +52,22 @@
 typedef unsigned short u16;
 typedef unsigned int u32x2 __attribute__((ext_vector_type(2)));
 typedef unsigned int u32x4 __attribute__((ext_vector_type(4)));
+
+__host__ __device__ inline float inv_sqrt_count(int c) { return 1.0f / sqrtf((float)c); }
+
+__host__ __device__ inline unsigned entry_word(int col, float dis, int col_bits) {
+  unsigned field = 0u;
+  if (dis > 0.0f && dis <= 1.0f) {
+    const double c = rint(1.0 / ((double)dis * (double)dis));
+    if (c >= 1.0 && c < (double)(1u << (32 - col_bits))) {
+      const int ci = (int)c;
+      if (__builtin_bit_cast(unsigned, inv_sqrt_count(ci)) == __builtin_bit_cast(unsigned, dis)) field = (unsigned)ci;
+    }
+  }
+  return ((unsigned)col & ((1u << col_bits) - 1u)) | (field << col_bits);
+}
+__host__ __device__ inline int entry_col(unsigned word, int col_bits) { return (int)(word & ((1u << col_bits) - 1u)); }
+__host__ __device__ inline int entry_count(unsigned word, int col_bits) { return (int)(word >> col_bits); }
 
 __device__ inline void lds_barrier() { asm volatile("s_waitcnt lgkmcnt(0)\n\ts_barrier" ::: "memory"); }
 
diff --git a/egc_amd/csrc/egc_graph.hip b/egc_amd/csrc/egc_graph.hip
--- a/egc_amd/csrc/egc_graph.hip
+++ b/egc_amd/csrc/egc_graph.hip
@@ -97,7 +97,7 @@
       for (int p = start + sl; p < end; p += 16) nonself += (col[p] != (int)row);
 #pragma unroll
       for (int off = 8; off > 0; off >>= 1) nonself += __shfl_xor(nonself, off);
-      if (live && sl == 0) dis_looped[row] = 1.0f / sqrtf((float)(nonself + 1));
+      if (live && sl == 0) dis_looped[row] = inv_sqrt_count(nonself + 1);
     }
     __syncthreads();
     for (int h = 0; h < s_huge_n; ++h) {
@@ -109,10 +109,10 @@
       for (int off = 32; off > 0; off >>= 1) nonself += __shfl_xor(nonself, off);
       if ((threadIdx.x & 63) == 0 && nonself != 0) atomicAdd(&s_huge_cnt[h], nonself);
       __syncthreads();
-      if (threadIdx.x == 0) dis_looped[hr] = 1.0f / sqrtf((float)(s_huge_cnt[h] + 1));
-    }
-  }
-  if (live && sl == 0 && dis_raw != nullptr) dis_raw[row] = deg > 0 ? 1.0f / sqrtf((float)deg) : 0.0f;
+      if (threadIdx.x == 0) dis_looped[hr] = inv_sqrt_count(s_huge_cnt[h] + 1);
+    }
+  }
+  if (live && sl == 0 && dis_raw != nullptr) dis_raw[row] = deg > 0 ? inv_sqrt_count(deg) : 0.0f;
   const bool is_long = live && deg > EGC_LONG_ROW_THRESHOLD;
   const int nch = is_long ? (deg + EGC_LONG_ROW_CHUNK - 1) / EGC_LONG_ROW_CHUNK : 0;
   int slot = 0, c0 = 0;
@@ -157,6 +157,17 @@
   }
 }
 
+__global__ void __launch_bounds__(256) pack_entries_kernel(int64_t n_edges, const int32_t* __restrict__ col,
+                                                           const float* __restrict__ edis_raw, const float* __restrict__ edis_looped,
+                                                           int col_bits, int32_t* __restrict__ out_raw, int32_t* __restrict__ out_looped) {
+  int64_t p = (int64_t)blockIdx.x * blockDim.x + threadIdx.x;
+  for (; p < n_edges; p += (int64_t)gridDim.x * blockDim.x) {
+    const int j = col[p];
+    if (out_raw != nullptr) out_raw[p] = (int32_t)entry_word(j, edis_raw[p], col_bits);
+    if (out_looped != nullptr) out_looped[p] = (int32_t)entry_word(j, edis_looped[p], col_bits);
+  }
+}
+
 __global__ void __launch_bounds__(256) csr_transposed_coo_kernel(int n_nodes, int64_t n_edges, const int32_t* __restrict__ rowptr,
                                                                  const int32_t* __restrict__ col, int64_t* __restrict__ out_src,
                                                                  int64_t* __restrict__ out_dst) {
@@ -336,8 +347,8 @@
   for (int k = 0; k < 4; ++k) {
     if (base + k < n_nodes) {
       rowptr[base + k] = run;
-      if (dis_raw != nullptr) dis_raw[base + k] = d[k] > 0 ? 1.0f / sqrtf((float)d[k]) : 0.0f;
-      if (dis_looped != nullptr) dis_looped[base + k] = 1.0f / sqrtf((float)(dn[k] + 1));
+      if (dis_raw != nullptr) dis_raw[base + k] = d[k] > 0 ? inv_sqrt_count(d[k]) : 0.0f;
+      if (dis_looped != nullptr) dis_looped[base + k] = inv_sqrt_count(dn[k] + 1);
       deg_ns[base + k] = 0;
       if (d[k] > EGC_LONG_ROW_THRESHOLD) {
         const int slot = atomicAdd(&plan[0], 1);
@@ -764,6 +775,41 @@
   const int blocks = (int)std::min<int64_t>(ceil_div(n_edges, 256), 256 * 8);
   edge_dis_kernel<<<blocks, 256, 0, stream>>>(n_edges, col, dis_raw, dis_looped, edge_dis_raw, edge_dis_looped);
   EGC_LAUNCH_CHECK("edge_dis_kernel");
+  return EGC_OK;
+}
+
+int32_t egc_entry_col_bits(int64_t n_src_rows) {
+  if (n_src_rows < 1 || n_src_rows > ((int64_t)1 << 31)) return 0;
+  int b = 1;
+  while (((int64_t)1 << b) < n_src_rows) ++b;
+  return b <= 30 ? b : 0;
+}
+
+int egc_csr_pack_entries(int64_t n_edges, const int32_t* col, const float* edge_dis_raw, const float* edge_dis_looped,
+                         int32_t col_bits, int32_t* entry_raw, int32_t* entry_looped, egc_stream_t stream_) {
+  hipStream_t stream = (hipStream_t)stream_;
+  if (n_edges < 0 || col_bits < 1 || col_bits > 30) return EGC_ERR_INVALID;
+  if (edge_dis_raw == nullptr) entry_raw = nullptr;
+  if (edge_dis_looped == nullptr) entry_looped = nullptr;
+  if (n_edges == 0 || (entry_raw == nullptr && entry_looped == nullptr)) return EGC_OK;
+  if (col == nullptr) return EGC_ERR_INVALID;
+  const int blocks = (int)std::min<int64_t>(ceil_div(n_edges, 256), 256 * 8);
+  pack_entries_kernel<<<blocks, 256, 0, stream>>>(n_edges, col, edge_dis_raw, edge_dis_looped, col_bits, entry_raw, entry_looped);
+  EGC_LAUNCH_CHECK("pack_entries_kernel");
+  return EGC_OK;
+}
+
+int egc_csr_pack_entries_host(int64_t n_edges, const int32_t* col, const float* edge_dis_raw, const float* edge_dis_looped,
+                              int32_t col_bits, int32_t* entry_raw, int32_t* entry_looped) {
+  if (n_edges < 0 || col_bits < 1 || col_bits > 30) return EGC_ERR_INVALID;
+  if (edge_dis_raw == nullptr) entry_raw = nullptr;
+  if (edge_dis_looped == nullptr) entry_looped = nullptr;
+  if (n_edges == 0 || (entry_raw == nullptr && entry_looped == nullptr)) return EGC_OK;
+  if (col == nullptr) return EGC_ERR_INVALID;
+  for (int64_t p = 0; p < n_edges; ++p) {
+    if (entry_raw != nullptr) entry_raw[p] = (int32_t)entry_word(col[p], edge_dis_raw[p], col_bits);
+    if (entry_looped != nullptr) entry_looped[p] = (int32_t)entry_word(col[p], edge_dis_looped[p], col_bits);
+  }
   return EGC_OK;
 }
 
diff --git a/egc_amd/graph.py b/egc_amd/graph.py
--- a/egc_amd/graph.py
+++ b/egc_amd/graph.py
@@ -73,6 +73,8 @@
         self.dis_raw, self.dis_looped, self.max_index, self.plan = dis_raw, dis_looped, max_index, plan
         self.device = rowptr.device
         self.edge_dis_raw = self.edge_dis_looped = None
+        self.entry_raw = self.entry_looped = None
+        self.entry_col_bits = 0
         self._workspaces = {}
         self._n_chunks = None
 
@@ -233,6 +235,27 @@
             _C.check(lib.egc_csr_edge_dis(e, self.col.data_ptr(), self.dis_raw.data_ptr(), self.dis_looped.data_ptr(),
                                           self.edge_dis_raw.data_ptr(), self.edge_dis_looped.data_ptr(),
                                           _stream_ptr(dev)), "egc_csr_edge_dis")
+        if self.entry_raw is not None:
+            self._pack_entries()
+
+    def _pack_entries(self):
+        lib = _C.load()
+        bits = int(lib.egc_entry_col_bits(self.n_src_rows))
+        if (self.halo is not None or self.n_src_rows != self.n_nodes or self.edge_dis_raw is None or self.n_edges == 0
+                or bits == 0):
+            self.entry_raw = self.entry_looped = None
+            self.entry_col_bits = 0
+            return
+        dev, e = self.device, self.n_edges
+        with _device_guard(dev):
+            if self.entry_raw is None:
+                e1 = (e + 3) & ~3
+                slab = torch.empty(2 * e1, dtype=torch.int32, device=dev)
+                self.entry_raw, self.entry_looped = slab[:e], slab[e1:e1 + e]
+            _C.check(lib.egc_csr_pack_entries(e, self.col.data_ptr(), self.edge_dis_raw.data_ptr(),
+                                              self.edge_dis_looped.data_ptr(), bits, self.entry_raw.data_ptr(),
+                                              self.entry_looped.data_ptr(), _stream_ptr(dev)), "egc_csr_pack_entries")
+        self.entry_col_bits = bits
 
     def transposed(self) -> "CSRGraph":
         if getattr(self, "_transposed", None) is None:
@@ -245,7 +268,7 @@
                                                           _stream_ptr(dev)), "egc_csr_transposed_coo")
                 self._transposed = CSRGraph.from_edge_index(coo, ns, max(n, 1), _poll=False)
         if self._n_chunks is not None and self._n_chunks >= 0:
-            self._transposed.trim_launches()
+            self._transposed.trim_launches(pack=False)
         return self._transposed
 
     def workspace(self, nbytes: int, zero_bytes: int | None = None) -> torch.Tensor:
@@ -269,19 +292,23 @@
                            self.edge_id.data_ptr(), self.dis_raw.data_ptr(), self.dis_looped.data_ptr(),
                            self.max_index.data_ptr(), self.plan.data_ptr(), self._n_chunks, self.n_src_rows,
                            self.edge_dis_raw.data_ptr() if self.edge_dis_raw is not None else None,
-                           self.edge_dis_looped.data_ptr() if self.edge_dis_looped is not None else None)
+                           self.edge_dis_looped.data_ptr() if self.edge_dis_looped is not None else None,
+                           self.entry_raw.data_ptr() if self.entry_raw is not None else None,
+                           self.entry_looped.data_ptr() if self.entry_looped is not None else None,
+                           self.entry_col_bits if self.entry_raw is not None else 0)
 
     def tensors(self) -> list:
         ts = [self.rowptr, self.col, self.edge_id, self.dis_raw, self.dis_looped, self.max_index, self.plan]
-        return ts + [t for t in (self.edge_dis_raw, self.edge_dis_looped) if t is not None]
+        return ts + [t for t in (self.edge_dis_raw, self.edge_dis_looped, self.entry_raw, self.entry_looped) if t is not None]
 
     def c_addr(self) -> int:
         key = (self._n_chunks, 0 if self.edge_dis_raw is None else self.edge_dis_raw.data_ptr(),
-               0 if self.edge_dis_looped is None else self.edge_dis_looped.data_ptr())
+               0 if self.edge_dis_looped is None else self.edge_dis_looped.data_ptr(),
+               0 if self.entry_raw is None else self.entry_raw.data_ptr())
         hit = getattr(self, "_c_cached", None)
         if hit is None or hit[0] != key or self._n_chunks is None:
             st = self.c_struct()
-            key = (self._n_chunks, key[1], key[2])
+            key = (self._n_chunks,) + key[1:]
             hit = self._c_cached = (key, st, C.addressof(st))
         else:
             _IndexFlag.poll()
@@ -300,10 +327,12 @@
             cache.setdefault("_keep", []).append(spec)
         return ws
 
-    def trim_launches(self) -> "CSRGraph":
+    def trim_launches(self, pack: bool = True) -> "CSRGraph":
         if self._n_chunks is None or self._n_chunks < 0:
             self._n_chunks = int(self.plan[1].item())
             self.check_indices()
+            if pack:
+                self._pack_entries()
         return self
 
     def long_row_stats(self):
diff --git a/include/egc_hip.h b/include/egc_hip.h
--- a/include/egc_hip.h
+++ b/include/egc_hip.h
@@ -51,6 +51,9 @@
   int64_t n_src_rows;
   const float* edge_dis_raw;
   const float* edge_dis_looped;
+  const int32_t* entry_raw;
+  const int32_t* entry_looped;
+  int32_t entry_col_bits;
 } egc_graph;
 
 int64_t egc_plan_ints(int64_t n_nodes, int64_t n_edges);
@@ -81,6 +84,12 @@
 
 int egc_csr_edge_dis(int64_t n_edges, const int32_t* col, const float* dis_raw, const float* dis_looped,
                      float* edge_dis_raw, float* edge_dis_looped, egc_stream_t stream);
+
+int32_t egc_entry_col_bits(int64_t n_src_rows);
+int egc_csr_pack_entries(int64_t n_edges, const int32_t* col, const float* edge_dis_raw, const float* edge_dis_looped,
+                         int32_t col_bits, int32_t* entry_raw, int32_t* entry_looped, egc_stream_t stream);
+int egc_csr_pack_entries_host(int64_t n_edges, const int32_t* col, const float* edge_dis_raw, const float* edge_dis_looped,
+                              int32_t col_bits, int32_t* entry_raw, int32_t* entry_looped);
 
 int egc_gather_rows_f32(const float* table, int64_t ld, const int64_t* idx, int64_t n_rows, int32_t width, float* out,
                         egc_stream_t stream);
```

Measured after the change: 18.59 billion edges/s (median of 6 runs). 1.01x the previous value.
